# antoinedesbois/Ray-Tracer-Rust

Measured on AMD Instinct MI355X. Metric: Mrays/sec + frame ms, big_bunny.obj @ 1920x1080, higher is better.
Workload: dtype f32

## Files before the change

include/rtx.h:

```cpp
#ifndef RTX_H
#define RTX_H

#include <stddef.h>
#include <stdint.h>

#ifdef __cplusplus
extern "C" {
#endif

#define RTX_ABI_VERSION 3

typedef enum RtxError {
    RTX_OK              =  0,
    RTX_ERR_BAD_ARG     = -1,
    RTX_ERR_NO_DEVICE   = -2,
    RTX_ERR_HIP         = -3,
    RTX_ERR_OOM         = -4,
    RTX_ERR_UNSUPPORTED = -5,
    RTX_ERR_INTERNAL    = -6,
    RTX_ERR_IO          = -7
} RtxError;

#define RTX_ACCEL_BVH    0u
#define RTX_ACCEL_BRUTE  1u
// ... 115 lines not shown
int rtx_render_view_rows(RtxScene *scene, int device, const RtxView *view, uint8_t *out_rgb, RtxStats *stats);
int rtx_render_view_rows_device(RtxScene *scene, int device, const RtxView *view, void *d_rgb, size_t d_bytes,
                                void *stream, uint64_t *d_counters);
int rtx_debug_aimed_nodes(RtxScene *scene, int device, const float eye[3], uint32_t *out_dwords);

typedef struct RtxLight {
    float v0[3], v1[3], v2[3];
    uint32_t nb_light_sample;
} RtxLight;

int rtx_scene_light(const RtxScene *scene, RtxLight *out);
int rtx_render_view_lit(RtxScene *scene, int device, const RtxView *view, const RtxLight *light, uint8_t *out_rgb,
                        RtxPixelShade *out_shade, RtxRayHit *out_hits, RtxStats *stats);
int rtx_render_view_lit_device(RtxScene *scene, int device, const RtxView *view, const RtxLight *light, void *d_rgb,
                               void *d_shade, void *d_hits, void *stream);
int rtx_shade_rays_lit(RtxScene *scene, int device, uint32_t n_pixels, const float *origins, const float *directions,
                       uint32_t flags, const RtxLight *light, RtxPixelShade *out_shade, RtxRayHit *out_hits ,
                       RtxStats *stats);
int rtx_shade_rays_lit_device(RtxScene *scene, int device, uint32_t n_pixels, const void *d_origins, const void *d_directions,
                              uint32_t flags, const RtxLight *light, void *d_shade, void *d_hits ,
                              void *stream);
int rtx_debug_light_points(RtxScene *scene, int device, const RtxLight *light, float *out);

int rtx_render_view_rows_lit(RtxScene *scene, int device, const RtxView *view, const RtxLight *light, uint8_t *out_rgb,
                             RtxStats *stats);
int rtx_render_view_rows_lit_device(RtxScene *scene, int device, const RtxView *view, const RtxLight *light, void *d_rgb,
                                    size_t d_bytes, void *stream, uint64_t *d_counters);
int rtx_debug_light_walk(RtxScene *scene, int device, const RtxLight *light, float *out_tour, float *out_boxes);

int rtx_scene_pose_bound(const RtxScene *scene, float *out_magnitude);
int rtx_scene_pose(RtxScene *scene, int device, const float *v0v1v2, const uint32_t *tie_rank ,
                   uint32_t reference_tree, RtxStats *stats);
int rtx_scene_pose_device(RtxScene *scene, int device, const void *d_v0v1v2, const void *d_tie_rank ,
                          void *stream);
int rtx_trace_rays_posed(RtxScene *scene, int device, uint32_t n_rays, const float *origins, const float *directions,
                         uint32_t flags, RtxRayHit *out_hits, RtxStats *stats);
int rtx_occluded_rays_posed(RtxScene *scene, int device, uint32_t n_rays, const float *origins, const float *targets,
                            uint32_t flags, uint8_t *out_occluded, RtxStats *stats);
int rtx_trace_rays_posed_device(RtxScene *scene, int device, uint32_t n_rays, const void *d_origins, const void *d_directions,
                                uint32_t flags, void *d_hits, void *stream);
int rtx_occluded_rays_posed_device(RtxScene *scene, int device, uint32_t n_rays, const void *d_origins, const void *d_targets,
                                   uint32_t flags, void *d_occluded, void *stream);
int rtx_shade_rays_posed(RtxScene *scene, int device, uint32_t n_pixels, const float *origins, const float *directions,
                         uint32_t flags, const RtxLight *light , RtxPixelShade *out_shade,
                         RtxRayHit *out_hits , RtxStats *stats);
int rtx_shade_rays_posed_device(RtxScene *scene, int device, uint32_t n_pixels, const void *d_origins, const void *d_directions,
                                uint32_t flags, const RtxLight *light , void *d_shade,
                                void *d_hits , void *stream);
int rtx_render_view_posed(RtxScene *scene, int device, const RtxView *view, const RtxLight *light ,
                          uint8_t *out_rgb, RtxPixelShade *out_shade, RtxRayHit *out_hits, RtxStats *stats);
int rtx_render_view_posed_device(RtxScene *scene, int device, const RtxView *view, const RtxLight *light ,
                                 void *d_rgb, void *d_shade, void *d_hits, void *stream);
int rtx_scene_posed_records(const RtxScene *scene, const float *v0v1v2, const uint32_t *tie_rank, uint32_t *out_tris,
                            uint32_t *out_shade, uint32_t *out_nodes);
int rtx_debug_pose(RtxScene *scene, int device, uint32_t *out_tris, uint32_t *out_shade, uint32_t *out_nodes);

int rtx_render_view_rows_posed(RtxScene *scene, int device, const RtxView *view, const RtxLight *light ,
                               uint8_t *out_rgb, RtxStats *stats);
int rtx_render_view_rows_posed_device(RtxScene *scene, int device, const RtxView *view, const RtxLight *light ,
                                      void *d_rgb, size_t d_bytes, void *stream, uint64_t *d_counters);
int rtx_scene_posed_pipeline_records(const RtxScene *scene, const float *v0v1v2, const float eye[3], uint32_t *out_planes,
                                     uint32_t *out_aimed);
int rtx_debug_pose_pipeline(RtxScene *scene, int device, const float eye[3], uint32_t *out_planes, uint32_t *out_aimed);

int rtx_scene_pose_rebuilt(RtxScene *scene, int device, const float *v0v1v2, const uint32_t *tie_rank ,
                           uint32_t reference_tree, RtxStats *stats);
int rtx_scene_pose_rebuilt_device(RtxScene *scene, int device, const void *d_v0v1v2, const void *d_tie_rank ,
                                  void *stream);
int rtx_scene_rebuilt_counts(const RtxScene *scene, uint32_t *out_n_nodes);
int rtx_scene_rebuilt_records(const RtxScene *scene, const float *v0v1v2, const uint32_t *tie_rank, uint64_t *out_keys,
                              uint32_t *out_perm, uint32_t *out_tris, uint32_t *out_shade, uint32_t *out_nodes);
int rtx_scene_rebuilt_aimed(const RtxScene *scene, const float *v0v1v2, const float eye[3], uint32_t *out_aimed);
int rtx_debug_pose_rebuilt(RtxScene *scene, int device, const float eye[3], uint32_t *out_perm, uint32_t *out_tris,
                           uint32_t *out_shade, uint32_t *out_nodes, uint32_t *out_aimed);

#define RTX_WAVE_PROFILE_WORDS 8
int rtx_debug_wave_profile(RtxScene *scene, int device, uint32_t row0, uint32_t nrows, uint64_t *out,
                           size_t out_tiles, uint32_t *tiles_x, uint32_t *tiles_y);

#define RTX_TIMING_RING 64
int rtx_launch_timings(RtxScene *scene, int device, int max_launches, float *schedule_ms, float *shade_ms);

int rtx_debug_tile_descs(RtxScene *scene, int device, uint32_t *out, size_t max_tiles);

const char *rtx_strerror(int err);
int rtx_last_hip_error(void);

int rtx_scene_light_points(const RtxScene *scene, float *out);
int rtx_scene_light_points_for(const RtxScene *scene, const RtxLight *light, float *out);
int rtx_scene_light_order(const RtxScene *scene, uint32_t *out);
int rtx_scene_light_walk_for(const RtxScene *scene, const RtxLight *light, uint32_t *out_order, float *out_boxes,
                             float *out_shaft_delta);
int rtx_scene_gamma_thresholds(const RtxScene *scene, float *out256);
int rtx_scene_normals(const RtxScene *scene, float *out);
int rtx_scene_nodes(const RtxScene *scene, uint32_t *out_dwords , uint32_t *out_tri_order );
int rtx_scene_primary_nodes(const RtxScene *scene, uint32_t *out_dwords , uint32_t *out_own);
int rtx_scene_aimed_nodes(const RtxScene *scene, const float eye[3], uint32_t *out_dwords);
int rtx_scene_ref_nodes(const RtxScene *scene, uint32_t *out_dwords);

void rtxh_camera_new(const float eye[3], const float look_at[3], const float up[3],
                     float u[3], float v[3], float w[3]);
int  rtxh_import_obj(const char *path, float **v0v1v2);
#define RTXH_OBJ_SLASHES   1u
#define RTXH_OBJ_RELATIVE  2u
#define RTXH_OBJ_POLYGONS  4u
#define RTXH_OBJ_MATERIALS 8u
#define RTXH_OBJ_ALL       15u
int  rtxh_import_obj_ex(const char *path, uint32_t flags, float **v0v1v2, float **rgb);
void rtxh_free(void *p);
int  rtxh_ref_leaf_rank(uint32_t n_tris, const float *v0v1v2, uint32_t *out_rank);
void rtxh_gen_samples(uint64_t seed, uint32_t n_pairs, float *out);
int  rtxh_scatter_tiles(uint8_t *frame, uint32_t height, uint32_t width, const uint8_t *packed, uint32_t first_tile,
                        uint32_t tile_stride, uint32_t tile_rows);
int  rtxh_write_png(const char *path, uint32_t width, uint32_t height, const uint8_t *rgb);
int  rtxh_synthetic_mesh(uint64_t seed, uint32_t n_tris, float *out_v0v1v2);

#ifdef __cplusplus
}
#endif
#endif
```

integration/rtx_ffi.rs:

```rust
#![allow(dead_code)]
use std::ffi::CStr;
use std::os::raw::{c_char, c_int, c_void};

pub const RTX_ABI_VERSION: c_int = 3;
pub const RTX_OK: c_int = 0;

#[repr(C)]
#[derive(Clone, Copy, Default)]
pub struct Sample {
    pub s0: f32,
    pub s1: f32,
}

#[repr(C)]
pub struct RtxSceneDesc {
    pub width: u32,
    pub height: u32,
    pub eye: [f32; 3],
    pub u: [f32; 3],
    pub v: [f32; 3],
    pub w: [f32; 3],
    pub distance: f32,
    pub light_v0: [f32; 3],
    pub light_v1: [f32; 3],
// ... 129 lines not shown
                           out_shade: *mut RtxPixelShade, out_hits: *mut RtxRayHit, stats: *mut RtxStats) -> c_int;
    pub fn rtx_render_view_device(scene: *mut RtxScene, device: c_int, view: *const RtxView, d_rgb: *mut c_void,
                                  d_shade: *mut c_void, d_hits: *mut c_void, stream: *mut c_void) -> c_int;
    pub fn rtx_render_view_rows(scene: *mut RtxScene, device: c_int, view: *const RtxView, out_rgb: *mut u8,
                                stats: *mut RtxStats) -> c_int;
    pub fn rtx_render_view_rows_device(scene: *mut RtxScene, device: c_int, view: *const RtxView, d_rgb: *mut c_void,
                                       d_bytes: usize, stream: *mut c_void, d_counters: *mut u64) -> c_int;
    pub fn rtx_scene_light(scene: *const RtxScene, out: *mut RtxLight) -> c_int;
    pub fn rtx_render_view_lit(scene: *mut RtxScene, device: c_int, view: *const RtxView, light: *const RtxLight,
                               out_rgb: *mut u8, out_shade: *mut RtxPixelShade, out_hits: *mut RtxRayHit,
                               stats: *mut RtxStats) -> c_int;
    pub fn rtx_render_view_lit_device(scene: *mut RtxScene, device: c_int, view: *const RtxView, light: *const RtxLight,
                                      d_rgb: *mut c_void, d_shade: *mut c_void, d_hits: *mut c_void,
                                      stream: *mut c_void) -> c_int;
    pub fn rtx_shade_rays_lit(scene: *mut RtxScene, device: c_int, n_pixels: u32, origins: *const f32,
                              directions: *const f32, flags: u32, light: *const RtxLight, out_shade: *mut RtxPixelShade,
                              out_hits: *mut RtxRayHit, stats: *mut RtxStats) -> c_int;
    pub fn rtx_shade_rays_lit_device(scene: *mut RtxScene, device: c_int, n_pixels: u32, d_origins: *const c_void,
                                     d_directions: *const c_void, flags: u32, light: *const RtxLight, d_shade: *mut c_void,
                                     d_hits: *mut c_void, stream: *mut c_void) -> c_int;
    pub fn rtx_scene_pose_bound(scene: *const RtxScene, out_magnitude: *mut f32) -> c_int;
    pub fn rtx_scene_pose(scene: *mut RtxScene, device: c_int, v0v1v2: *const f32, tie_rank: *const u32, reference_tree: u32,
                          stats: *mut RtxStats) -> c_int;
    pub fn rtx_scene_pose_device(scene: *mut RtxScene, device: c_int, d_v0v1v2: *const c_void, d_tie_rank: *const c_void,
                                 stream: *mut c_void) -> c_int;
    pub fn rtx_trace_rays_posed(scene: *mut RtxScene, device: c_int, n_rays: u32, origins: *const f32, directions: *const f32,
                                flags: u32, out_hits: *mut RtxRayHit, stats: *mut RtxStats) -> c_int;
    pub fn rtx_occluded_rays_posed(scene: *mut RtxScene, device: c_int, n_rays: u32, origins: *const f32, targets: *const f32,
                                   flags: u32, out_occluded: *mut u8, stats: *mut RtxStats) -> c_int;
    pub fn rtx_trace_rays_posed_device(scene: *mut RtxScene, device: c_int, n_rays: u32, d_origins: *const c_void,
                                       d_directions: *const c_void, flags: u32, d_hits: *mut c_void,
                                       stream: *mut c_void) -> c_int;
    pub fn rtx_occluded_rays_posed_device(scene: *mut RtxScene, device: c_int, n_rays: u32, d_origins: *const c_void,
                                          d_targets: *const c_void, flags: u32, d_occluded: *mut c_void,
                                          stream: *mut c_void) -> c_int;
    pub fn rtx_shade_rays_posed(scene: *mut RtxScene, device: c_int, n_pixels: u32, origins: *const f32, directions: *const f32,
                                flags: u32, light: *const RtxLight, out_shade: *mut RtxPixelShade, out_hits: *mut RtxRayHit,
                                stats: *mut RtxStats) -> c_int;
    pub fn rtx_shade_rays_posed_device(scene: *mut RtxScene, device: c_int, n_pixels: u32, d_origins: *const c_void,
                                       d_directions: *const c_void, flags: u32, light: *const RtxLight, d_shade: *mut c_void,
                                       d_hits: *mut c_void, stream: *mut c_void) -> c_int;
    pub fn rtx_render_view_posed(scene: *mut RtxScene, device: c_int, view: *const RtxView, light: *const RtxLight,
                                 out_rgb: *mut u8, out_shade: *mut RtxPixelShade, out_hits: *mut RtxRayHit,
                                 stats: *mut RtxStats) -> c_int;
    pub fn rtx_render_view_posed_device(scene: *mut RtxScene, device: c_int, view: *const RtxView, light: *const RtxLight,
                                        d_rgb: *mut c_void, d_shade: *mut c_void, d_hits: *mut c_void,
                                        stream: *mut c_void) -> c_int;
    pub fn rtx_scene_posed_records(scene: *const RtxScene, v0v1v2: *const f32, tie_rank: *const u32, out_tris: *mut u32,
                                   out_shade: *mut u32, out_nodes: *mut u32) -> c_int;
    pub fn rtx_debug_pose(scene: *mut RtxScene, device: c_int, out_tris: *mut u32, out_shade: *mut u32,
                          out_nodes: *mut u32) -> c_int;
    pub fn rtx_render_view_rows_posed(scene: *mut RtxScene, device: c_int, view: *const RtxView, light: *const RtxLight,
                                      out_rgb: *mut u8, stats: *mut RtxStats) -> c_int;
    pub fn rtx_render_view_rows_posed_device(scene: *mut RtxScene, device: c_int, view: *const RtxView, light: *const RtxLight,
                                             d_rgb: *mut c_void, d_bytes: usize, stream: *mut c_void,
                                             d_counters: *mut u64) -> c_int;
    pub fn rtx_scene_posed_pipeline_records(scene: *const RtxScene, v0v1v2: *const f32, eye: *const f32, out_planes: *mut u32,
                                            out_aimed: *mut u32) -> c_int;
    pub fn rtx_debug_pose_pipeline(scene: *mut RtxScene, device: c_int, eye: *const f32, out_planes: *mut u32,
                                   out_aimed: *mut u32) -> c_int;
    pub fn rtx_scene_pose_rebuilt(scene: *mut RtxScene, device: c_int, v0v1v2: *const f32, tie_rank: *const u32,
                                  reference_tree: u32, stats: *mut RtxStats) -> c_int;
    pub fn rtx_scene_pose_rebuilt_device(scene: *mut RtxScene, device: c_int, d_v0v1v2: *const c_void, d_tie_rank: *const c_void,
                                         stream: *mut c_void) -> c_int;
    pub fn rtx_scene_rebuilt_counts(scene: *const RtxScene, out_n_nodes: *mut u32) -> c_int;
    pub fn rtx_scene_rebuilt_records(scene: *const RtxScene, v0v1v2: *const f32, tie_rank: *const u32, out_keys: *mut u64,
                                     out_perm: *mut u32, out_tris: *mut u32, out_shade: *mut u32, out_nodes: *mut u32) -> c_int;
    pub fn rtx_scene_rebuilt_aimed(scene: *const RtxScene, v0v1v2: *const f32, eye: *const f32, out_aimed: *mut u32) -> c_int;
    pub fn rtx_debug_pose_rebuilt(scene: *mut RtxScene, device: c_int, eye: *const f32, out_perm: *mut u32, out_tris: *mut u32,
                                  out_shade: *mut u32, out_nodes: *mut u32, out_aimed: *mut u32) -> c_int;
    pub fn rtx_scene_light_points_for(scene: *const RtxScene, light: *const RtxLight, out: *mut f32) -> c_int;
    pub fn rtx_debug_light_points(scene: *mut RtxScene, device: c_int, light: *const RtxLight, out: *mut f32) -> c_int;
    pub fn rtx_render_view_rows_lit(scene: *mut RtxScene, device: c_int, view: *const RtxView, light: *const RtxLight,
                                    out_rgb: *mut u8, stats: *mut RtxStats) -> c_int;
    pub fn rtx_render_view_rows_lit_device(scene: *mut RtxScene, device: c_int, view: *const RtxView, light: *const RtxLight,
                                           d_rgb: *mut c_void, d_bytes: usize, stream: *mut c_void,
                                           d_counters: *mut u64) -> c_int;
    pub fn rtx_scene_light_walk_for(scene: *const RtxScene, light: *const RtxLight, out_order: *mut u32, out_boxes: *mut f32,
                                    out_shaft_delta: *mut f32) -> c_int;
    pub fn rtx_debug_light_walk(scene: *mut RtxScene, device: c_int, light: *const RtxLight, out_tour: *mut f32,
                                out_boxes: *mut f32) -> c_int;
    pub fn rtx_launch_timings(scene: *mut RtxScene, device: c_int, max_launches: c_int, schedule_ms: *mut f32,
                              shade_ms: *mut f32) -> c_int;
    pub fn rtx_strerror(err: c_int) -> *const c_char;
    pub fn rtx_last_hip_error() -> c_int;
    pub fn rtxh_scatter_tiles(frame: *mut u8, height: u32, width: u32, packed: *const u8, first_tile: u32,
                              tile_stride: u32, tile_rows: u32) -> c_int;
    pub fn rtxh_camera_new(eye: *const f32, look_at: *const f32, up: *const f32, u: *mut f32, v: *mut f32, w: *mut f32);
    pub fn rtxh_ref_leaf_rank(n_tris: u32, v0v1v2: *const f32, out_rank: *mut u32) -> c_int;
}

pub fn check(rc: c_int) -> Result<(), String> {
    if rc == RTX_OK {
        Ok(())
    } else {
        let text = unsafe { CStr::from_ptr(rtx_strerror(rc)) };
        Err(format!("librtx: {} [{}]", text.to_string_lossy(), rc))
    }
}
```

ray-tracer-rust_amd/csrc/rtx_api.cpp:

```cpp
#include <hip/hip_runtime.h>

#include <algorithm>
#include <chrono>
#include <cmath>
#include <cstddef>
#include <cstdio>
#include <cstdlib>
#include <cstring>
#include <initializer_list>
#include <map>
#include <memory>
#include <mutex>
#include <new>
#include <vector>

#include "../../include/rtx.h"
#include "rtx_aim.h"
#include "rtx_device.h"
#include "rtx_light.h"
#include "rtx_planes.h"
#include "rtx_pose.h"
#include "rtx_rebuild.h"
#include "rtx_query.h"
#include "rtx_shade.h"
#include "rtx_tour.h"
#include "rtx_view.h"
#include "scene_prep.h"

namespace {

thread_local int g_last_hip_error = 0;

int hip_rc(hipError_t e)
{
    if (e == hipSuccess) return RTX_OK;
    g_last_hip_error = static_cast<int>(e);
    return e == hipErrorOutOfMemory ? RTX_ERR_OOM : RTX_ERR_HIP;
}

#define RTX_TRY(step)                          \
    do {                                       \
        const int rc_ = (step);                \
        if (rc_ != RTX_OK) return rc_;         \
    } while (0)
#define RTX_HIP(call) RTX_TRY(hip_rc(call))

class DeviceGuard {
public:
    DeviceGuard() = default;
    explicit DeviceGuard(int dev) { (void)set(dev); }
    ~DeviceGuard() { if (ok_) (void)hipSetDevice(prev_); }
    hipError_t set(int dev) { ok_ = hipGetDevice(&prev_) == hipSuccess; return err_ = hipSetDevice(dev); }
    hipError_t status() const { return err_; }
private:
    int prev_ = 0;
    bool ok_ = false;
    hipError_t err_ = hipSuccess;
};

template <class T, hipError_t (*Free)(T)>
class Owned {
public:
    Owned() = default;
    Owned(const Owned &) = delete;
    Owned &operator=(const Owned &) = delete;
    ~Owned() { (void)reset(); }
    hipError_t reset()
    {
        const hipError_t e = h_ ? Free(h_) : hipSuccess;
        h_ = nullptr;
        return e;
    }
    T *put() { return &h_; }
    operator T() const { return h_; }
private:
    T h_ = nullptr;
};
using Stream = Owned<hipStream_t, hipStreamDestroy>;
using Event = Owned<hipEvent_t, hipEventDestroy>;

int mark_busy(Event &e, hipStream_t callers)
{
    if (!e) RTX_HIP(hipEventCreateWithFlags(e.put(), hipEventDisableTiming));
    RTX_HIP(hipEventRecord(e, callers));
    return RTX_OK;
}

int wait_for(const Event &e, hipStream_t stream)
{
    if (e) RTX_HIP(hipStreamWaitEvent(stream, e, 0));
    return RTX_OK;
}

hipError_t alloc_device(void **p, size_t bytes) { return hipMalloc(p, bytes); }
hipError_t alloc_pinned(void **p, size_t bytes) { return hipHostMalloc(p, bytes, hipHostMallocDefault); }

template <hipError_t (*Alloc)(void **, size_t), hipError_t (*Free)(void *)>
class GrowOnly {
public:
    int reserve(size_t bytes)
    {
        if (cap_ >= bytes) return RTX_OK;
        cap_ = 0;
        RTX_HIP(mem_.reset());
        RTX_HIP(Alloc(mem_.put(), bytes));
        cap_ = bytes;
        return RTX_OK;
    }
    size_t capacity() const { return cap_; }
    template <class T>
    T *as() const { return static_cast<T *>(static_cast<void *>(mem_)); }
private:
    Owned<void *, Free> mem_;
    size_t cap_ = 0;
};
using DeviceBuffer = GrowOnly<alloc_device, hipFree>;
using PinnedBuffer = GrowOnly<alloc_pinned, hipHostFree>;

struct Sized { DeviceBuffer &buffer; size_t bytes; };
int reserve_all(std::initializer_list<Sized> list)
{
    for (const Sized &s : list) {
        const int rc = s.buffer.reserve(s.bytes);
        if (rc != RTX_OK) return rc;
    }
    return RTX_OK;
}

struct AimedStream {
    DeviceBuffer nodes, links;
    float eye[3] = {0.0f, 0.0f, 0.0f};
    hipStream_t on = nullptr;
    bool valid = false;
};

struct DeviceGeometry {
    DeviceBuffer nodes, ref_nodes, tris, shade, planes;
    uint32_t n_nodes = 0;
    uint32_t n_ref_nodes = 0;
    AimedStream aimed;
};

class DeviceState {
public:
    explicit DeviceState(int dev) : device(dev) {}
    const int device;
    bool uploaded = false;
    size_t last_tiles = 0;
    unsigned long long launches = 0;
    Stream stream;
    Event ev0, ev1;
    Event ring[RTX_TIMING_RING][3];
    Event q_sorted;
    DeviceGeometry geo;
    DeviceBuffer primary_nodes, samples, lights, light_tour, thr, light_boxes;
    DeviceBuffer d_out, d_counters;
    DeviceBuffer d_redo;
    bool launch_words_ready = false;
    uint32_t words_launches = 0, words_passes = 0;
    PinnedBuffer h_stage;
    struct { DeviceBuffer hits, pix_slot, tiles, chunks, results, acc, ctr, buckets, cut; } ws;
    DeviceBuffer q_first, q_second, q_out;
    struct { DeviceBuffer keys, keys_sorted, index, index_sorted, temp; } q_sort;
    struct {
        DeviceBuffer points, tour, boxes;
        Event used;
    } lit;
    struct {
        DeviceBuffer tri_of, ranges, order;
        bool tables = false;
        DeviceBuffer v, rank;
        DeviceGeometry geo;
        bool valid = false;
        Event used;
        struct {
            DeviceBuffer nodes, ranges, order;
            bool tables = false;
            DeviceBuffer keys, keys_sorted, index, perm, temp;
        } b;
        bool rebuilt = false;
    } pose;
private:
    ~DeviceState() = default;
    friend struct ReleaseOnDevice;
};

struct ReleaseOnDevice {
    void operator()(DeviceState *st) const
    {
        DeviceGuard g(st->device);
        if (g.status() != hipSuccess) return;
        if (st->stream) (void)hipStreamSynchronize(st->stream);
        delete st;
    }
};

struct DeviceSlot {
    std::mutex mu;
    std::unique_ptr<DeviceState, ReleaseOnDevice> st;
};

enum : unsigned { kUsesSort = 1u, kUsesLight = 2u, kUsesPose = 4u };

int wait_for_uses(DeviceState &st, unsigned uses)
{
    if (uses & kUsesSort) RTX_TRY(wait_for(st.q_sorted, st.stream));
    if (uses & kUsesLight) RTX_TRY(wait_for(st.lit.used, st.stream));
    if (uses & kUsesPose) RTX_TRY(wait_for(st.pose.used, st.stream));
    return RTX_OK;
}

int mark_uses(DeviceState &st, unsigned uses, hipStream_t callers)
{
    if (uses & kUsesSort) RTX_TRY(mark_busy(st.q_sorted, callers));
    if (uses & kUsesLight) RTX_TRY(mark_busy(st.lit.used, callers));
    if (uses & kUsesPose) RTX_TRY(mark_busy(st.pose.used, callers));
    return RTX_OK;
}

double wall_ms()
{
    using namespace std::chrono;
    return duration<double, std::milli>(steady_clock::now().time_since_epoch()).count();
}

}

struct RtxScene {
    rtx::PreparedScene prep;
    std::mutex mu;
    rtx::PoseTables pose_tables;
    bool pose_tables_made = false;
    rtx::RebuildTables rebuild_tables;
    bool rebuild_tables_made = false;
    std::map<int, DeviceSlot> dev;
};

namespace {

int device_count_quiet()
{
    int n = 0;
    if (hipGetDeviceCount(&n) != hipSuccess) return 0;
    return n < 0 ? 0 : n;
}

int get_slot(RtxScene *scene, int device, DeviceSlot **out)
{
    if (device < 0 || device >= device_count_quiet()) return RTX_ERR_NO_DEVICE;
    std::lock_guard<std::mutex> lk(scene->mu);
    *out = &scene->dev[device];
    return RTX_OK;
}

int ensure_state(DeviceSlot &slot, int device)
{
    if (!slot.st) slot.st.reset(new (std::nothrow) DeviceState(device));
    return slot.st ? RTX_OK : RTX_ERR_OOM;
}

template <class T>
int upload_vec(DeviceBuffer &dst, const std::vector<T> &v, size_t pad_bytes = 0)
{
    const size_t bytes = v.size() * sizeof(T);
    const int rc = dst.reserve(bytes + pad_bytes ? bytes + pad_bytes : 16);
    if (rc != RTX_OK) return rc;
    if (bytes) RTX_HIP(hipMemcpy(dst.as<void>(), v.data(), bytes, hipMemcpyHostToDevice));
    if (pad_bytes) RTX_HIP(hipMemset(dst.as<char>() + bytes, 0, pad_bytes));
    return RTX_OK;
}

uint32_t kernel_variant()
{
#if RTX_ABLATION
    static const uint32_t v = [] {
        const char *e = std::getenv("RTX_VARIANT");
        return e ? static_cast<uint32_t>(std::atoi(e)) & rtx::kVariantMask : rtx::kDefaultVariant;
    }();
    return v;
#else
    return rtx::kDefaultVariant;
#endif
}

int upload_all(RtxScene *scene, DeviceState &st)
{
    const rtx::PreparedScene &p = scene->prep;
    int rc;
    const float inflate = p.cull_delta;
    DeviceGeometry &g = st.geo;
    if ((rc = upload_vec(g.nodes, rtx::nodes_in_device_order(p.nodes, inflate), sizeof(rtx::NodeRec))) != RTX_OK) return rc;
    if (!p.primary_nodes.empty() &&
        (rc = upload_vec(st.primary_nodes, rtx::nodes_in_device_order(p.primary_nodes, inflate), sizeof(rtx::NodeRec))) != RTX_OK) return rc;
    if (!p.ref_nodes.empty() &&
        (rc = upload_vec(g.ref_nodes, rtx::nodes_in_device_order(p.ref_nodes), sizeof(rtx::NodeRec))) != RTX_OK) return rc;
    g.n_nodes = static_cast<uint32_t>(p.nodes.size());
    g.n_ref_nodes = static_cast<uint32_t>(p.ref_nodes.size());
    if ((rc = upload_vec(g.tris, p.tris, sizeof(rtx::TriRec))) != RTX_OK) return rc;
    if ((rc = upload_vec(g.shade, p.shade)) != RTX_OK) return rc;
    if ((rc = upload_vec(st.samples, p.samples)) != RTX_OK) return rc;
    if ((rc = upload_vec(st.lights, p.light_points)) != RTX_OK) return rc;
    if ((rc = upload_vec(st.light_tour, p.light_tour)) != RTX_OK) return rc;
    if (!p.global_planes.empty() && (rc = upload_vec(g.planes, p.global_planes)) != RTX_OK) return rc;
    if ((rc = upload_vec(st.light_boxes, p.light_boxes)) != RTX_OK) return rc;
    if ((rc = st.thr.reserve(sizeof(p.gamma_thr))) != RTX_OK) return rc;
    RTX_HIP(hipMemcpy(st.thr.as<void>(), p.gamma_thr, sizeof(p.gamma_thr), hipMemcpyHostToDevice));
    if ((rc = st.d_counters.reserve(rtx::kNumCounters * sizeof(unsigned long long))) != RTX_OK) return rc;
    RTX_HIP(hipStreamCreateWithFlags(st.stream.put(), hipStreamNonBlocking));
    RTX_HIP(hipEventCreate(st.ev0.put()));
    RTX_HIP(hipEventCreate(st.ev1.put()));
    for (auto &slot : st.ring)
        for (Event &e : slot) RTX_HIP(hipEventCreate(e.put()));
    st.uploaded = true;
    return RTX_OK;
}

int ensure_uploaded(RtxScene *scene, DeviceSlot &slot)
{
    if (slot.st->uploaded) return RTX_OK;
    const int rc = upload_all(scene, *slot.st);
    if (rc != RTX_OK) slot.st.reset();
    return rc;
}

class Entry {
public:
    enum Need { kLocked, kCurrent, kUploaded };
    Entry(RtxScene *scene, int device, Need need)
    {
        if ((rc = get_slot(scene, device, &slot)) != RTX_OK) return;
        lock_ = std::unique_lock<std::mutex>(slot->mu);
        if ((rc = ensure_state(*slot, device)) != RTX_OK) return;
        if (need >= kCurrent && (rc = make_current()) != RTX_OK) return;
        if (need >= kUploaded) rc = ensure_uploaded(scene, *slot);
    }
    int make_current() { return hip_rc(guard_.set(slot->st->device)); }
    DeviceState &state() const { return *slot->st; }
    int rc = RTX_ERR_INTERNAL;
    DeviceSlot *slot = nullptr;
private:
    std::unique_lock<std::mutex> lock_;
    DeviceGuard guard_;
};

int geometry_of(DeviceState &st, bool posed, DeviceGeometry **out)
{
    *out = &st.geo;
    if (!posed) return RTX_OK;
    if (!st.pose.valid) return RTX_ERR_BAD_ARG;
    *out = &st.pose.geo;
    return RTX_OK;
}

rtx::DeviceScene device_scene(const RtxScene *scene, const DeviceState &st, const DeviceGeometry &g)
{
    const rtx::PreparedScene &p = scene->prep;
    rtx::DeviceScene S;
    S.nodes = g.nodes.as<const rtx::NodeRec>();
    S.primary_nodes = st.primary_nodes.capacity() ? st.primary_nodes.as<const rtx::NodeRec>() : st.geo.nodes.as<const rtx::NodeRec>();
    S.light_tour = st.light_tour.as<const float>();
    S.n_wide = 0u;
    S.ref_nodes = g.ref_nodes.as<const rtx::NodeRec>();
    S.n_ref_nodes = g.n_ref_nodes;
    S.tris = g.tris.as<const rtx::TriRec>();
    S.shade = g.shade.as<const rtx::ShadeRec>();
    S.samples = st.samples.as<const float2>();
    S.light_points = st.lights.as<const float>();
    S.planes = g.planes.as<const rtx::TriRec>();
    S.gamma_thr = st.thr.as<const float>();
    S.light_boxes = st.light_boxes.as<const float>();
    S.shaft_delta = p.shaft_delta;
    S.n_nodes = g.n_nodes;
    S.n_samples = p.n_samples;
    S.width = p.width;
    S.height = p.height;
    S.nb_ray = p.nb_ray;
    S.nb_light = p.nb_light_sample;
    S.n_spheres = p.n_spheres;
    S.n_global = p.n_global;
    std::memcpy(S.eye, p.eye, 12);
    std::memcpy(S.cu, p.cam_u, 12);
    std::memcpy(S.cv, p.cam_v, 12);
    std::memcpy(S.cw, p.cam_w, 12);
    S.distance = p.distance;
    S.cut_max_nodes = rtx::kCutMaxNodes;
    S.n_prims = static_cast<uint32_t>(p.tris.size());
    S.j1_mode = 0u;
// ... 5 lines not shown
        if (m == 1u || ((m == 2u || m == 3u) && p.n_spheres == 0u)) S.j1_mode = m;
    }
#endif
    return S;
}

int reserve_stream_ws(DeviceState &st, const rtx::DeviceScene &S, const rtx::TileSpec &ts, rtx::StreamWorkspace *ws, bool *used)
{
    *used = (kernel_variant() & (rtx::kVariantStream | rtx::kVariantProbe)) != 0u;
    if (!*used) return RTX_OK;
    const rtx::StreamWorkspaceBytes need = rtx::stream_workspace_bytes(S, ts, kernel_variant());
    const int rc = reserve_all({{st.ws.hits, need.hits}, {st.ws.pix_slot, need.pix_slot}, {st.ws.tiles, need.tiles},
                                {st.ws.chunks, need.chunks}, {st.ws.results, need.results}, {st.ws.acc, need.acc},
                                {st.ws.ctr, need.ctr}, {st.ws.buckets, need.buckets}, {st.ws.cut, need.cut}});
    if (rc != RTX_OK) return rc;
    st.last_tiles = need.tiles / sizeof(rtx::TileDesc);
    *ws = rtx::StreamWorkspace{st.ws.hits.as<rtx::HitRec>(), st.ws.pix_slot.as<uint32_t>(), st.ws.tiles.as<rtx::TileDesc>(),
                               st.ws.chunks.as<uint2>(), st.ws.results.as<float>(), st.ws.acc.as<float>(),
                               st.ws.ctr.as<uint32_t>(), st.ws.buckets.as<uint32_t>(), st.ws.cut.as<rtx::CutEntry>()};
    return RTX_OK;
}

uint32_t tiles_rows(uint32_t height, uint32_t first_tile, uint32_t tile_stride, uint32_t tile_rows)
{
    if (!tile_rows || !tile_stride) return 0;
    uint64_t rows = 0;
    for (uint64_t t = first_tile; t * tile_rows < height; t += tile_stride) {
        const uint64_t r0 = t * tile_rows;
        rows += (height - r0 < tile_rows) ? (height - r0) : tile_rows;
    }
    return static_cast<uint32_t>(rows);
}

void fill_stats(RtxStats *s, uint64_t primary_rays, uint32_t shadow_rays_per_hit, const unsigned long long *c,
                double kernel_ms, double total_ms)
{
    std::memset(s, 0, sizeof *s);
    s->primary_rays = primary_rays;
    s->primary_hits = c[0];
    s->shadow_rays = c[0] * shadow_rays_per_hit;
    s->rays = s->primary_rays + s->shadow_rays;
    s->box_tests = c[1];
    s->tri_tests = c[2];
    s->wave_node_visits = c[3];
    s->wave_tri_visits = c[4];
    s->redo_tiles = c[5];
    s->kernel_ms = kernel_ms;
    s->total_ms = total_ms;
}

struct Timed {
    explicit Timed(RtxStats *s) : stats(s) {}
    RtxStats *const stats;
    const double t0 = wall_ms();
    unsigned long long *counters(const DeviceState &st) const { return stats ? st.d_counters.as<unsigned long long>() : nullptr; }
    int empty() const
    {
        const unsigned long long none[rtx::kNumCounters] = {0};
        if (stats) fill_stats(stats, 0, 0, none, 0.0, wall_ms() - t0);
        return RTX_OK;
    }
    int begin(const DeviceState &st) const
    {
        if (stats) RTX_HIP(hipMemsetAsync(counters(st), 0, rtx::kNumCounters * sizeof(unsigned long long), st.stream));
        RTX_HIP(hipEventRecord(st.ev0, st.stream));
        return RTX_OK;
    }
    int end(const DeviceState &st) const { return hip_rc(hipEventRecord(st.ev1, st.stream)); }
    int gather(const DeviceState &st, uint64_t primary_rays, uint32_t shadow_rays_per_hit) const
    {
        unsigned long long c[rtx::kNumCounters] = {0};
        if (stats) RTX_HIP(hipMemcpyAsync(c, counters(st), sizeof c, hipMemcpyDeviceToHost, st.stream));
        RTX_HIP(hipStreamSynchronize(st.stream));
        if (!stats) return RTX_OK;
        float ms = 0.0f;
        RTX_HIP(hipEventElapsedTime(&ms, st.ev0, st.ev1));
        fill_stats(stats, primary_rays, shadow_rays_per_hit, c, ms, wall_ms() - t0);
        return RTX_OK;
    }
};

template <class Before>
int render_launch(DeviceState &st, const rtx::DeviceScene &S, const rtx::TileSpec &ts, uint8_t *d_out,
                  unsigned long long *d_counters, unsigned long long *d_wave_prof, hipStream_t stream, Before before)
{
    int rc;
    const size_t redo_cap = st.d_redo.capacity(), buckets_cap = st.ws.buckets.capacity();
    if ((rc = st.d_redo.reserve(rtx::trace_redo_bytes(S, ts))) != RTX_OK) return rc;
    rtx::StreamWorkspace ws{};
    bool use_ws = false;
    if (!d_wave_prof && (rc = reserve_stream_ws(st, S, ts, &ws, &use_ws)) != RTX_OK) return rc;
    if ((rc = before()) != RTX_OK) return rc;
    const Event *slot = st.ring[st.launches % RTX_TIMING_RING];
    hipEvent_t phases[3] = {slot[0], slot[1], slot[2]};
    const bool two_pass = use_ws && (kernel_variant() & rtx::kVariantProbe) != 0u && ts.local_rows != 0u;
    if (two_pass && (!st.launch_words_ready || st.d_redo.capacity() != redo_cap || st.ws.buckets.capacity() != buckets_cap)) {
        RTX_HIP(rtx::zero_launch_words(st.d_redo.as<uint32_t>(), ws, stream));
        st.words_launches = st.words_passes = 0;
    }
    if (ts.local_rows) st.launch_words_ready = false;
    RTX_HIP(rtx::launch_trace_shade(S, ts, d_out, st.d_redo.as<uint32_t>(), use_ws ? &ws : nullptr, d_counters, d_wave_prof,
                                    kernel_variant(), stream, d_wave_prof ? nullptr : phases, st.words_launches, st.words_passes));
    if (two_pass) {
        st.launch_words_ready = true;
        ++st.words_launches;
        st.words_passes += S.nb_ray;
    }
    if (!d_wave_prof && ts.local_rows) ++st.launches;
    return RTX_OK;
}

int launch_on(RtxScene *scene, DeviceSlot &slot, const rtx::TileSpec &ts, const Timed &timed)
{
    RTX_TRY(ensure_uploaded(scene, slot));
    DeviceState &st = *slot.st;
    const size_t bytes = static_cast<size_t>(ts.local_rows) * scene->prep.width * 3u;
    RTX_TRY(st.d_out.reserve(bytes ? bytes : 16));
    RTX_TRY(render_launch(st, device_scene(scene, st, st.geo), ts, st.d_out.as<uint8_t>(), timed.counters(st), nullptr, st.stream,
                          [&] { return timed.begin(st); }));
    return timed.end(st);
}


uint32_t tree_root(const rtx::PreparedScene &p, size_t n_nodes)
{
    return (p.n_global != 0u && n_nodes > 2u) ? 2u : 0u;
}
uint32_t tree_root(const rtx::PreparedScene &p) { return tree_root(p, p.nodes.size()); }

float origin_bound(const RtxScene *scene) { return scene->prep.cull_delta * 0x1p19f; }

rtxq::KeyBox query_key_box(const rtx::PreparedScene &p)
{
    rtxq::KeyBox box{};
    if (p.nodes.empty()) return box;
    const rtx::NodeRec &root = p.nodes[tree_root(p)];
    for (int a = 0; a < 3; ++a) {
        const float extent = root.bmax[a] - root.bmin[a];
        const float scale = static_cast<float>(1u << rtxq::kMortonBitsPerAxis) / extent;
        box.lo[a] = root.bmin[a];
        box.scale[a] = (extent > 0.0f && scale > 0.0f && scale < 0x1p100f) ? scale : 0.0f;
    }
    return box;
}

int reserve_query_sort(DeviceState &st, uint32_t n, rtxq::SortBuffers *sort)
{
    const size_t words = static_cast<size_t>(n) * sizeof(uint32_t);
    size_t temp = 0;
    RTX_HIP(rtxq::sort_temp_bytes(n, &temp));
    const int rc = reserve_all({{st.q_sort.keys, words}, {st.q_sort.keys_sorted, words}, {st.q_sort.index, words},
                                {st.q_sort.index_sorted, words}, {st.q_sort.temp, temp ? temp : 16}});
    if (rc != RTX_OK) return rc;
    *sort = rtxq::SortBuffers{st.q_sort.keys.as<uint32_t>(), st.q_sort.keys_sorted.as<uint32_t>(), st.q_sort.index.as<uint32_t>(),
                              st.q_sort.index_sorted.as<uint32_t>(), st.q_sort.temp.as<void>(), st.q_sort.temp.capacity()};
    return RTX_OK;
}

static_assert(sizeof(RtxRayHit) == 32, "closest_kernel writes a hit as two 16-byte words");
static_assert(sizeof(RtxPixelShade) == 16, "shade_kernel writes a pixel as one 16-byte word");
static_assert(sizeof(RtxView) == sizeof(rtxv::ViewBlock) && alignof(RtxView) == 4, "view_kernel is handed an RtxView");
constexpr uint32_t kQueryFlags = RTX_RAYS_KEEP_ORDER | RTX_RAYS_FORCE_REGROUP;

uint32_t shade_ray_count(const RtxScene *scene, uint32_t n_pixels)
{
    const uint64_t n = static_cast<uint64_t>(n_pixels) * scene->prep.nb_ray;
    return n <= rtxq::kMaxRays ? static_cast<uint32_t>(n) : 0u;
}

constexpr int kBatchOuts = 3;
struct BatchArgs {
    rtx::DeviceScene S;
    uint32_t n;
    const float *first, *second;
    const RtxView *view;
    rtxq::KeyBox box;
    float origin_bound;
    const rtxq::SortBuffers *sort;
    void *out[kBatchOuts];
    unsigned long long *counters;
    hipStream_t stream;
};

template <bool Occlusion>
hipError_t launch_queried(const BatchArgs &a)
{
    return rtxq::launch_query(a.S, Occlusion, a.n, a.first, a.second, a.box, a.origin_bound, a.sort, a.out[0], a.counters, a.stream);
}

hipError_t launch_shaded(const BatchArgs &a)
{
    return rtxs::launch_shade(a.S, a.n, a.first, a.second, a.box, a.origin_bound, a.sort, a.out[0], a.out[1], a.counters, a.stream);
}

enum { kViewShade, kViewHits, kViewRgb };

hipError_t launch_viewed(const BatchArgs &a)
{
    rtxv::ViewBlock v;
    std::memcpy(&v, a.view, sizeof v);
    return rtxv::launch_view(a.S, v, a.origin_bound, a.out[kViewRgb], a.out[kViewShade], a.out[kViewHits], a.counters, a.stream);
}
// ... 397 lines not shown

int shade_host(RtxScene *scene, int device, uint32_t n_pixels, const float *origins, const float *directions, uint32_t flags,
               const Lit *lit, bool posed, RtxPixelShade *shade, RtxRayHit *hits, RtxStats *stats)
{
    if (!shade_args_ok(scene, origins, directions, shade, flags, n_pixels)) return RTX_ERR_BAD_ARG;
    return batch_host(scene, device, shade_batch(scene, n_pixels, flags, lit, posed, hits != nullptr), origins, directions,
                      {shade, hits, nullptr}, stats);
}

int shade_device(RtxScene *scene, int device, uint32_t n_pixels, const void *d_origins, const void *d_directions, uint32_t flags,
                 const Lit *lit, bool posed, void *d_shade, void *d_hits, void *stream)
{
    if (!shade_args_ok(scene, d_origins, d_directions, d_shade, flags, n_pixels) || !aligned16(d_shade, d_hits)) return RTX_ERR_BAD_ARG;
    return batch_device(scene, device, shade_batch(scene, n_pixels, flags, lit, posed, d_hits != nullptr), d_origins, d_directions,
                        {d_shade, d_hits, nullptr}, stream);
}


bool eye_in_pipeline_range(const RtxScene *scene, const float eye[3])
{
    const float bound = origin_bound(scene);
    for (int k = 0; k < 3; ++k)
        if (!(std::fabs(eye[k]) <= bound)) return false;
    return true;
}

bool view_rows_args_ok(const RtxScene *scene, const RtxView *v, const void *out)
{
    if (!scene || !v || !out || !frame_ok(v)) return false;
    if (v->x0 != 0u || v->nx != v->width) return false;
    return static_cast<uint64_t>(v->y0) + v->ny <= v->height;
}

int reserve_aimed(const RtxScene *scene, DeviceGeometry &g)
{
    if (scene->prep.primary_nodes.empty()) return RTX_OK;
    AimedStream &a = g.aimed;
    const size_t n = g.n_nodes;
    const size_t had = a.nodes.capacity();
    const int rc = reserve_all({{a.nodes, (n + 1u) * sizeof(rtx::NodeDev)}, {a.links, n * sizeof(rtxa::AimLink)}});
    if (rc != RTX_OK || a.nodes.capacity() != had) a.valid = false;
    return rc;
}

const rtx::NodeRec *aimed_stream(const RtxScene *scene, const DeviceGeometry &g)
{
    return (scene->prep.primary_nodes.empty() ? g.nodes : g.aimed.nodes).as<const rtx::NodeRec>();
}

int aim_at(const RtxScene *scene, DeviceGeometry &g, const float eye[3], hipStream_t stream)
{
    const rtx::PreparedScene &p = scene->prep;
    if (p.primary_nodes.empty()) return RTX_OK;
    AimedStream &a = g.aimed;
    if (a.valid && a.on == stream && std::memcmp(a.eye, eye, 12) == 0) return RTX_OK;
    a.valid = false;
    const uint32_t n = g.n_nodes;
    RTX_HIP(hipMemsetAsync(a.nodes.as<rtx::NodeDev>() + n, 0, sizeof(rtx::NodeDev), stream));
    RTX_HIP(rtxa::launch_aim(g.nodes.as<const rtx::NodeDev>(), n, tree_root(p, n), eye, a.links.as<rtxa::AimLink>(),
                             a.nodes.as<rtx::NodeDev>(), stream));
    std::memcpy(a.eye, eye, 12);
    a.on = stream;
    a.valid = true;
    return RTX_OK;
}

template <class Before>
int view_rows_launch(RtxScene *scene, DeviceState &st, DeviceGeometry &g, const RtxView &v, uint8_t *d_out,
                     unsigned long long *d_counters, hipStream_t stream, Before before, const Lit *lit, float shaft_delta)
{
    RTX_TRY(reserve_aimed(scene, g));
    if (lit) RTX_TRY(reserve_light(scene, st, *lit, true));
    rtx::DeviceScene S = device_scene(scene, st, g);
    if (lit) light_swap(st, *lit, true, shaft_delta, &S);
    S.width = v.width;
    S.height = v.height;
    std::memcpy(S.eye, v.eye, 12);
    std::memcpy(S.cu, v.u, 12);
    std::memcpy(S.cv, v.v, 12);
    std::memcpy(S.cw, v.w, 12);
    S.distance = v.distance;
    S.primary_nodes = aimed_stream(scene, g);
    const rtx::TileSpec ts{v.y0, v.ny, v.ny, v.ny};
    return render_launch(st, S, ts, d_out, d_counters, nullptr, stream, [&]() -> int {
        RTX_TRY(before());
        RTX_TRY(aim_at(scene, g, v.eye, stream));
        return lit ? light_launch(scene, st, *lit, true, stream) : RTX_OK;
    });
}

int view_rows_supported(const RtxScene *scene, const RtxView *view, const Lit *lit, float *shaft_delta)
{
    if (!eye_in_pipeline_range(scene, view->eye)) return RTX_ERR_UNSUPPORTED;
    return lit ? lit_rows_margin(scene, *lit, shaft_delta) : RTX_OK;
}

int view_rows_host(RtxScene *scene, int device, const RtxView *view, const Lit *lit, bool posed, uint8_t *out_rgb, RtxStats *stats)
{
    if (!view_rows_args_ok(scene, view, out_rgb)) return RTX_ERR_BAD_ARG;
    const Timed timed(stats);
    if (view->ny == 0u) return timed.empty();
    float shaft_delta = 0.0f;
    RTX_TRY(view_rows_supported(scene, view, lit, &shaft_delta));
    Entry e(scene, device, Entry::kUploaded);
    if (e.rc != RTX_OK) return e.rc;
    DeviceState &st = e.state();
    const RtxView v = *view;
    const size_t bytes = static_cast<size_t>(v.ny) * v.width * 3u;
    RTX_TRY(st.d_out.reserve(bytes));
    DeviceGeometry *geo;
    RTX_TRY(geometry_of(st, posed, &geo));
    RTX_TRY(wait_for_uses(st, uses_of(lit, posed)));
    RTX_TRY(view_rows_launch(scene, st, *geo, v, st.d_out.as<uint8_t>(), timed.counters(st), st.stream, [&] { return timed.begin(st); },
                             lit, shaft_delta));
    RTX_TRY(timed.end(st));
    RTX_HIP(hipMemcpyAsync(out_rgb, st.d_out.as<void>(), bytes, hipMemcpyDeviceToHost, st.stream));
    return timed.gather(st, static_cast<uint64_t>(v.ny) * v.width * scene->prep.nb_ray, lit ? lit->count : scene->prep.nb_light_sample);
}

int view_rows_device(RtxScene *scene, int device, const RtxView *view, const Lit *lit, bool posed, void *d_rgb, size_t d_bytes,
                     void *stream, uint64_t *d_counters)
{
    if (!view_rows_args_ok(scene, view, d_rgb)) return RTX_ERR_BAD_ARG;
    if (d_bytes < static_cast<size_t>(view->ny) * view->width * 3u) return RTX_ERR_BAD_ARG;
    if (view->ny == 0u) return RTX_OK;
    float shaft_delta = 0.0f;
    RTX_TRY(view_rows_supported(scene, view, lit, &shaft_delta));
    Entry e(scene, device, Entry::kUploaded);
    if (e.rc != RTX_OK) return e.rc;
    DeviceGeometry *geo;
    RTX_TRY(geometry_of(e.state(), posed, &geo));
    RTX_TRY(view_rows_launch(scene, e.state(), *geo, *view, static_cast<uint8_t *>(d_rgb), reinterpret_cast<unsigned long long *>(d_counters),
                             static_cast<hipStream_t>(stream), [] { return static_cast<int>(RTX_OK); }, lit, shaft_delta));
    return mark_uses(e.state(), uses_of(lit, posed), static_cast<hipStream_t>(stream));
}

void posed_pipeline_on_host(RtxScene *scene, const float *pose, const float *eye, rtx::TriRec *planes, rtx::NodeRec *aimed)
{
    const rtx::PreparedScene &p = scene->prep;
    const rtx::PoseTables &t = pose_tables_of(scene);
    std::vector<rtx::TriRec> tris(p.tris.size());
    std::vector<rtx::NodeRec> nodes(aimed ? p.nodes.size() : 0u);
    rtx::posed_records(p, t, pose, nullptr, tris.data(), nullptr, aimed ? nodes.data() : nullptr);
    if (planes)
        for (uint32_t i = 0; i < p.n_global; ++i) rtx::global_plane_statement(tris[i], planes + i);
    if (!aimed) return;
    if (!p.primary_nodes.empty()) {
        std::vector<rtx::NodeRec> out;
        rtx::stream_nearest_first(nodes, tree_root(p), eye, out);
        nodes.swap(out);
    }
    std::memcpy(aimed, nodes.data(), nodes.size() * sizeof(rtx::NodeRec));
}

std::vector<rtx::NodeRec> aimed_on_host(const rtx::PreparedScene &p, const float eye[3])
{
    std::vector<rtx::NodeRec> moved(p.nodes);
    const float inflate = p.cull_delta;
    for (rtx::NodeRec &n : moved)
        for (int k = 0; k < 3; ++k) {
            n.bmin[k] = n.bmin[k] - inflate;
            n.bmax[k] = n.bmax[k] + inflate;
        }
    if (p.primary_nodes.empty()) return moved;
    std::vector<rtx::NodeRec> out;
    rtx::stream_nearest_first(moved, tree_root(p), eye, out);
// ... 219 lines not shown
        RTX_HIP(g.status());
        const auto &n = need[kv.second];
        int rc = ensure_state(*kv.second, kv.first);
        if (rc != RTX_OK) return rc;
        if ((rc = kv.second->st->d_out.reserve(n.first ? n.first : 16)) != RTX_OK) return rc;
        if ((rc = kv.second->st->h_stage.reserve(n.second ? n.second : 16)) != RTX_OK) return rc;
    }
    unsigned long long total[rtx::kNumCounters] = {0};
    std::vector<unsigned long long> counters(static_cast<size_t>(n_devices) * rtx::kNumCounters, 0ull);
    std::vector<float> share_ms(static_cast<size_t>(n_devices), 0.0f);
    for (int j = 0; j < n_devices; ++j) {
        Share &sh = shares[j];
        if (!sh.spec.local_rows) continue;
        DeviceGuard g(devices[j]);
        if (g.status() != hipSuccess) return fail(hip_rc(g.status()));
        const int rc = launch_on(scene, *sh.slot, sh.spec, Timed(stats));
        if (rc != RTX_OK) return fail(rc);
        launched.push_back(devices[j]);
        DeviceState &st = *sh.slot->st;
        hipError_t e = hipMemcpyAsync(st.h_stage.as<uint8_t>() + sh.stage_offset, st.d_out.as<void>(), sh.spec.local_rows * row_bytes,
                                      hipMemcpyDeviceToHost, st.stream);
        if (e == hipSuccess && stats)
            e = hipMemcpyAsync(&counters[static_cast<size_t>(j) * rtx::kNumCounters], st.d_counters.as<void>(),
                               rtx::kNumCounters * sizeof(unsigned long long), hipMemcpyDeviceToHost, st.stream);
        if (e != hipSuccess) return fail(hip_rc(e));
        if (stats && unique.size() != static_cast<size_t>(n_devices)) {
            if ((e = hipStreamSynchronize(st.stream)) != hipSuccess || (e = hipEventElapsedTime(&share_ms[j], st.ev0, st.ev1)) != hipSuccess)
                return fail(hip_rc(e));
        }
    }
    double kernel_ms = 0.0;
    for (auto &kv : unique) {
        DeviceGuard g(kv.first);
        if (g.status() != hipSuccess) return fail(hip_rc(g.status()));
        const hipError_t e = hipStreamSynchronize(kv.second->st->stream);
        if (e != hipSuccess) return fail(hip_rc(e));
    }
    for (int j = 0; j < n_devices; ++j) {
        const Share &sh = shares[j];
        if (!sh.spec.local_rows) continue;
        rtxh_scatter_tiles(out_rgb, H, W, sh.slot->st->h_stage.as<uint8_t>() + sh.stage_offset, static_cast<uint32_t>(j), static_cast<uint32_t>(n_devices), tile_rows);
        if (stats) {
            if (unique.size() == static_cast<size_t>(n_devices)) {
                DeviceGuard g(devices[j]);
                float ms = 0.0f;
                if (g.status() == hipSuccess && hipEventElapsedTime(&ms, sh.slot->st->ev0, sh.slot->st->ev1) == hipSuccess) share_ms[j] = ms;
            }
            for (int k = 0; k < rtx::kNumCounters; ++k) total[k] += counters[static_cast<size_t>(j) * rtx::kNumCounters + k];
        }
    }
    if (stats) {
        std::map<DeviceSlot *, double> per_device;
        for (int j = 0; j < n_devices; ++j) per_device[shares[j].slot] += share_ms[j];
        for (auto &kv : per_device) kernel_ms = std::max(kernel_ms, kv.second);
        fill_stats(stats, static_cast<uint64_t>(H) * W * scene->prep.nb_ray, scene->prep.nb_light_sample, total, kernel_ms, wall_ms() - t0);
    }
    return RTX_OK;
}

uint32_t rtx_tiles_rows(const RtxScene *scene, uint32_t first_tile, uint32_t tile_stride, uint32_t tile_rows)
{
    return scene ? tiles_rows(scene->prep.height, first_tile, tile_stride, tile_rows) : 0;
}

size_t rtx_tiles_bytes(const RtxScene *scene, uint32_t first_tile, uint32_t tile_stride, uint32_t tile_rows)
{
    return scene ? static_cast<size_t>(tiles_rows(scene->prep.height, first_tile, tile_stride, tile_rows)) *
                       scene->prep.width * 3u
                 : 0;
}

int rtx_render_tiles_device(RtxScene *scene, int device, uint32_t first_tile, uint32_t tile_stride,
                            uint32_t tile_rows, void *d_out_rgb, size_t d_out_bytes, void *stream,
                            uint64_t *d_counters)
{
    if (!scene || !d_out_rgb || !tile_rows || !tile_stride) return RTX_ERR_BAD_ARG;
    const uint32_t rows = tiles_rows(scene->prep.height, first_tile, tile_stride, tile_rows);
    if (static_cast<size_t>(rows) * scene->prep.width * 3u > d_out_bytes) return RTX_ERR_BAD_ARG;
    if (static_cast<uint64_t>(first_tile) * tile_rows > 0xFFFFFFFFull ||
        static_cast<uint64_t>(tile_stride) * tile_rows > 0xFFFFFFFFull) return RTX_ERR_BAD_ARG;
    Entry e(scene, device, Entry::kUploaded);
    if (e.rc != RTX_OK) return e.rc;
    const rtx::TileSpec ts{first_tile * tile_rows, tile_rows, tile_stride * tile_rows, rows};
    return render_launch(e.state(), device_scene(scene, e.state(), e.state().geo), ts, static_cast<uint8_t *>(d_out_rgb),
                         reinterpret_cast<unsigned long long *>(d_counters), nullptr, static_cast<hipStream_t>(stream),
                         [] { return static_cast<int>(RTX_OK); });
}

int rtx_trace_rays(RtxScene *scene, int device, uint32_t n_rays, const float *origins, const float *directions,
                   uint32_t flags, RtxRayHit *out_hits, RtxStats *stats)
{
    if (!query_args_ok(scene, origins, directions, out_hits, flags, n_rays)) return RTX_ERR_BAD_ARG;
    return batch_host(scene, device, query_batch(false, n_rays, flags, false), origins, directions, {out_hits, nullptr, nullptr}, stats);
}

int rtx_occluded_rays(RtxScene *scene, int device, uint32_t n_rays, const float *origins, const float *targets,
                      uint32_t flags, uint8_t *out_occluded, RtxStats *stats)
{
    if (!query_args_ok(scene, origins, targets, out_occluded, flags, n_rays)) return RTX_ERR_BAD_ARG;
    return batch_host(scene, device, query_batch(true, n_rays, flags, false), origins, targets, {out_occluded, nullptr, nullptr}, stats);
}

int rtx_trace_rays_device(RtxScene *scene, int device, uint32_t n_rays, const void *d_origins, const void *d_directions,
                          uint32_t flags, void *d_hits, void *stream)
{
    if (!query_args_ok(scene, d_origins, d_directions, d_hits, flags, n_rays) || !aligned16(d_hits)) return RTX_ERR_BAD_ARG;
    return batch_device(scene, device, query_batch(false, n_rays, flags, false), d_origins, d_directions, {d_hits, nullptr, nullptr}, stream);
}

int rtx_occluded_rays_device(RtxScene *scene, int device, uint32_t n_rays, const void *d_origins, const void *d_targets,
                             uint32_t flags, void *d_occluded, void *stream)
{
    if (!query_args_ok(scene, d_origins, d_targets, d_occluded, flags, n_rays)) return RTX_ERR_BAD_ARG;
    return batch_device(scene, device, query_batch(true, n_rays, flags, false), d_origins, d_targets, {d_occluded, nullptr, nullptr}, stream);
}

int rtx_shade_rays(RtxScene *scene, int device, uint32_t n_pixels, const float *origins, const float *directions,
                   uint32_t flags, RtxPixelShade *out_shade, RtxRayHit *out_hits, RtxStats *stats)
{
    return shade_host(scene, device, n_pixels, origins, directions, flags, nullptr, false, out_shade, out_hits, stats);
}

int rtx_shade_rays_device(RtxScene *scene, int device, uint32_t n_pixels, const void *d_origins, const void *d_directions,
                          uint32_t flags, void *d_shade, void *d_hits, void *stream)
{
    return shade_device(scene, device, n_pixels, d_origins, d_directions, flags, nullptr, false, d_shade, d_hits, stream);
}

int rtx_scene_view(const RtxScene *scene, RtxView *out)
{
    if (!scene || !out) return RTX_ERR_BAD_ARG;
    const rtx::PreparedScene &p = scene->prep;
    std::memset(out, 0, sizeof *out);
    out->width = out->nx = p.width;
    out->height = out->ny = p.height;
    std::memcpy(out->eye, p.eye, 12);
    std::memcpy(out->u, p.cam_u, 12);
    std::memcpy(out->v, p.cam_v, 12);
    std::memcpy(out->w, p.cam_w, 12);
    out->distance = p.distance;
    return RTX_OK;
}

int rtx_render_view(RtxScene *scene, int device, const RtxView *view, uint8_t *out_rgb, RtxPixelShade *out_shade,
                    RtxRayHit *out_hits, RtxStats *stats)
{
    return view_host(scene, device, view, nullptr, false, out_rgb, out_shade, out_hits, stats);
}

int rtx_render_view_device(RtxScene *scene, int device, const RtxView *view, void *d_rgb, void *d_shade, void *d_hits,
                           void *stream)
{
    return view_device(scene, device, view, nullptr, false, d_rgb, d_shade, d_hits, stream);
}

int rtx_scene_light(const RtxScene *scene, RtxLight *out)
{
    if (!scene || !out) return RTX_ERR_BAD_ARG;
    const rtx::PreparedScene &p = scene->prep;
    std::memcpy(out->v0, p.light_v, 12);
    std::memcpy(out->v1, p.light_v + 3, 12);
    std::memcpy(out->v2, p.light_v + 6, 12);
    out->nb_light_sample = p.nb_light_sample;
    return RTX_OK;
}

int rtx_render_view_lit(RtxScene *scene, int device, const RtxView *view, const RtxLight *light, uint8_t *out_rgb,
                        RtxPixelShade *out_shade, RtxRayHit *out_hits, RtxStats *stats)
{
// ... 342 lines not shown
    if (!scene || !v0v1v2 || (out_aimed && !eye)) return RTX_ERR_BAD_ARG;
    try {
        posed_pipeline_on_host(const_cast<RtxScene *>(scene), v0v1v2, eye, reinterpret_cast<rtx::TriRec *>(out_planes),
                               reinterpret_cast<rtx::NodeRec *>(out_aimed));
    } catch (...) {
        return RTX_ERR_OOM;
    }
    return RTX_OK;
}

int rtx_debug_pose_pipeline(RtxScene *scene, int device, const float eye[3], uint32_t *out_planes, uint32_t *out_aimed)
{
    if (!scene || (out_aimed && !eye)) return RTX_ERR_BAD_ARG;
    Entry e(scene, device, Entry::kUploaded);
    if (e.rc != RTX_OK) return e.rc;
    DeviceState &st = e.state();
    DeviceGeometry *g;
    RTX_TRY(geometry_of(st, true, &g));
    if (st.pose.rebuilt && out_aimed) return RTX_ERR_BAD_ARG;
    const size_t n = scene->prep.nodes.size(), n_global = scene->prep.n_global;
    RTX_TRY(wait_for_uses(st, kUsesPose));
    if (out_planes && n_global)
        RTX_HIP(hipMemcpyAsync(out_planes, g->planes.as<void>(), n_global * sizeof(rtx::TriRec), hipMemcpyDeviceToHost, st.stream));
    if (out_aimed && n) {
        RTX_TRY(reserve_aimed(scene, *g));
        g->aimed.valid = false;
        RTX_TRY(aim_at(scene, *g, eye, st.stream));
    }
    return read_back_nodes(st, aimed_stream(scene, *g), n, out_aimed);
}

int rtx_debug_wave_profile(RtxScene *scene, int device, uint32_t row0, uint32_t nrows, uint64_t *out,
                           size_t out_tiles, uint32_t *tiles_x, uint32_t *tiles_y)
{
    if (!scene || !tiles_x || !tiles_y) return RTX_ERR_BAD_ARG;
    const uint32_t H = scene->prep.height;
    if (row0 > H || nrows > H - row0 || nrows == 0) return RTX_ERR_BAD_ARG;
#if !RTX_ABLATION
    (void)device; (void)out; (void)out_tiles;
    return RTX_ERR_UNSUPPORTED;
#else
    Entry en(scene, device, Entry::kUploaded);
    if (en.rc != RTX_OK) return en.rc;
    DeviceState &st = en.state();
    const rtx::DeviceScene S = device_scene(scene, st, st.geo);
    *tiles_x = rtx::trace_tiles_x(S, kernel_variant());
    *tiles_y = (nrows + 7u) / 8u;
    const size_t n = static_cast<size_t>(*tiles_x) * *tiles_y;
    if (!out) return RTX_OK;
    if (out_tiles < n) return RTX_ERR_BAD_ARG;
    int rc = st.d_out.reserve(static_cast<size_t>(nrows) * scene->prep.width * 3u);
    if (rc != RTX_OK) return rc;
    unsigned long long *d_prof = nullptr;
    const size_t prof_bytes = n * rtx::kWaveProfWords * sizeof(unsigned long long);
    RTX_HIP(hipMalloc(reinterpret_cast<void **>(&d_prof), prof_bytes));
    const rtx::TileSpec ts{row0, nrows, nrows, nrows};
    rc = render_launch(st, S, ts, st.d_out.as<uint8_t>(), nullptr, d_prof, st.stream,
                       [&] { return hip_rc(hipMemsetAsync(d_prof, 0, prof_bytes, st.stream)); });
    if (rc == RTX_OK) rc = hip_rc(hipMemcpyAsync(out, d_prof, prof_bytes, hipMemcpyDeviceToHost, st.stream));
    if (rc == RTX_OK) rc = hip_rc(hipStreamSynchronize(st.stream));
    (void)hipFree(d_prof);
    if (rc != RTX_OK) return rc;
    for (size_t t = 0; t < n; ++t)
        out[rtx::kWaveProfWords * t + 2] = ~out[rtx::kWaveProfWords * t + 2];
    return RTX_OK;
#endif
}

int rtx_debug_tile_descs(RtxScene *scene, int device, uint32_t *out, size_t max_tiles)
{
    if (!scene) return RTX_ERR_BAD_ARG;
    Entry e(scene, device, Entry::kLocked);
    if (e.rc != RTX_OK) return e.rc;
    const DeviceState &st = e.state();
    if (!out) return static_cast<int>(st.last_tiles);
    const int rc = e.make_current();
    if (rc != RTX_OK) return rc;
    const size_t n = st.last_tiles < max_tiles ? st.last_tiles : max_tiles;
    RTX_HIP(hipDeviceSynchronize());
    if (n) RTX_HIP(hipMemcpy(out, st.ws.tiles.as<void>(), n * sizeof(rtx::TileDesc), hipMemcpyDeviceToHost));
    return static_cast<int>(n);
}

int rtx_launch_timings(RtxScene *scene, int device, int max_launches, float *schedule_ms, float *shade_ms)
{
    if (!scene || max_launches < 0 || !schedule_ms || !shade_ms) return RTX_ERR_BAD_ARG;
    Entry e(scene, device, Entry::kCurrent);
    if (e.rc != RTX_OK) return e.rc;
    const DeviceState &st = e.state();
    unsigned long long n = st.launches < RTX_TIMING_RING ? st.launches : RTX_TIMING_RING;
    if (n > static_cast<unsigned long long>(max_launches)) n = static_cast<unsigned long long>(max_launches);
    for (unsigned long long i = 0; i < n; ++i) {
        const Event *ev = st.ring[(st.launches - n + i) % RTX_TIMING_RING];
        RTX_HIP(hipEventSynchronize(ev[2]));
        RTX_HIP(hipEventElapsedTime(&schedule_ms[i], ev[0], ev[1]));
        RTX_HIP(hipEventElapsedTime(&shade_ms[i], ev[1], ev[2]));
    }
    return static_cast<int>(n);
}

int rtx_scene_light_points(const RtxScene *scene, float *out)
{
    if (!scene || !out) return RTX_ERR_BAD_ARG;
    std::memcpy(out, scene->prep.light_points.data(), scene->prep.light_points.size() * sizeof(float));
    return RTX_OK;
}

int rtx_scene_light_order(const RtxScene *scene, uint32_t *out)
{
    if (!scene || !out) return RTX_ERR_BAD_ARG;
    std::memcpy(out, scene->prep.light_order.data(), scene->prep.light_order.size() * sizeof(uint32_t));
    return RTX_OK;
}

int rtx_scene_gamma_thresholds(const RtxScene *scene, float *out256)
{
    if (!scene || !out256) return RTX_ERR_BAD_ARG;
    std::memcpy(out256, scene->prep.gamma_thr, sizeof scene->prep.gamma_thr);
    return RTX_OK;
}

int rtx_scene_normals(const RtxScene *scene, float *out)
{
    if (!scene || !out) return RTX_ERR_BAD_ARG;
    for (size_t i = 0; i < scene->prep.shade.size(); ++i) std::memcpy(out + 3 * i, scene->prep.shade[i].normal, 12);
    return RTX_OK;
}

int rtx_scene_ref_nodes(const RtxScene *scene, uint32_t *out_dwords)
{
    if (!scene || !out_dwords) return RTX_ERR_BAD_ARG;
    std::memcpy(out_dwords, scene->prep.ref_nodes.data(), scene->prep.ref_nodes.size() * sizeof(rtx::NodeRec));
    return RTX_OK;
}

int rtx_scene_primary_nodes(const RtxScene *scene, uint32_t *out_dwords, uint32_t *out_own)
{
    if (!scene) return RTX_ERR_BAD_ARG;
    const bool own = !scene->prep.primary_nodes.empty();
    const std::vector<rtx::NodeRec> &v = own ? scene->prep.primary_nodes : scene->prep.nodes;
    if (out_dwords) std::memcpy(out_dwords, v.data(), v.size() * sizeof(rtx::NodeRec));
    if (out_own) *out_own = own ? 1u : 0u;
    return RTX_OK;
}

int rtx_scene_nodes(const RtxScene *scene, uint32_t *out_dwords, uint32_t *out_tri_order)
{
    if (!scene) return RTX_ERR_BAD_ARG;
    if (out_dwords)
        std::memcpy(out_dwords, scene->prep.nodes.data(), scene->prep.nodes.size() * sizeof(rtx::NodeRec));
    if (out_tri_order)
        for (size_t i = 0; i < scene->prep.tris.size(); ++i) out_tri_order[i] = scene->prep.tris[i].idx;
    return RTX_OK;
}

}
```

ray-tracer-rust_amd/csrc/rtx_device.h:

```cpp
#pragma once

#include <hip/hip_runtime.h>

#include <cstdint>

#include "scene_prep.h"

#ifndef RTX_ABLATION
#define RTX_ABLATION 0
#endif

namespace rtx {

struct DeviceScene {
    const NodeRec  *nodes;
    const NodeRec  *primary_nodes;
    const float    *light_tour;
    const NodeRec  *ref_nodes;
    const TriRec   *tris;
    const ShadeRec *shade;
    const TriRec   *planes;
    const float2   *samples;
    const float    *light_points;
    const float    *gamma_thr;
    const float    *light_boxes;
    uint32_t n_nodes, n_ref_nodes, n_samples, n_wide;
    uint32_t width, height;
    uint32_t nb_ray, nb_light;
    uint32_t n_global;
    uint32_t n_spheres;
    float eye[3], cu[3], cv[3], cw[3];
    float distance;
    float shaft_delta;
    uint32_t cut_max_nodes;
    uint32_t n_prims;
    uint32_t j1_mode;
};
constexpr uint32_t kCutMaxNodes = 1u << 16;

struct TileSpec {
    uint32_t first_row;
    uint32_t tile_rows;
    uint32_t tile_stride_rows;
    uint32_t local_rows;
};

struct TileDesc {
    uint32_t first;
    uint32_t n_hit;
    uint32_t flags;
    uint32_t pad;
};
struct HitRec {
    float p[3], n[3], rgb[3], pad[3];
};
static_assert(sizeof(TileDesc) == 16 && sizeof(HitRec) == 48, "stream record sizes");
struct CutEntry {
    uint32_t begin, end;
    NodeDev  root;
};
static_assert(sizeof(CutEntry) == 40, "CutEntry is ten dwords");
constexpr uint32_t kCutWords = sizeof(CutEntry) / 4u;
#ifndef RTX_MAX_CUT
#define RTX_MAX_CUT 16
#endif
constexpr uint32_t kMaxCut = RTX_MAX_CUT;
struct StreamWorkspace {
    HitRec   *hits;
    uint32_t *pix_slot;
    TileDesc *tiles;
    uint2    *chunks;
    float    *results;
    float    *acc;
    uint32_t *ctr;
    uint32_t *buckets;
    CutEntry *cut;
};
constexpr uint32_t kCutInnerFlag = 1u << 29, kCutEndMask = (1u << 26) - 1u;
constexpr uint32_t kCutStreamRecords = kMaxCut + 1u;
__host__ __device__ inline size_t cut_stream_offset(size_t tiles)
{
    return (tiles * kMaxCut * sizeof(CutEntry) + 63u) & ~static_cast<size_t>(63u);
}
struct StreamWorkspaceBytes { size_t hits, pix_slot, tiles, chunks, results, acc, ctr, buckets, cut; };
static_assert(kMaxCut >= 1u && kMaxCut <= 51u && kCutWords * kMaxCut <= 512u, "RTX_MAX_CUT: 1 .. 51 (one staged word per work-item of 512)");
constexpr uint32_t kTileCutShift = 8u;
constexpr uint32_t kTileCompactHits = 8u;
constexpr uint32_t kTileChunk0Kept = 4u;
StreamWorkspaceBytes stream_workspace_bytes(const DeviceScene &S, const TileSpec &ts, uint32_t variant);
constexpr uint32_t kCostBuckets = 64u;
constexpr uint32_t kStreamCtrWords = 4u;

constexpr int kNumCounters = 8;


constexpr uint32_t kVariantStream = 8u;
constexpr uint32_t kVariantPacked = 16u;
constexpr uint32_t kVariantProbe = 32u;
constexpr uint32_t kVariantMask = 63u;
constexpr uint32_t kDefaultVariant = kVariantProbe | 1u;

constexpr size_t kWaveProfWords = 8;
uint32_t trace_tiles_x(const DeviceScene &S, uint32_t variant);
constexpr uint32_t kQueueRedoCount = 0u, kQueueNextTile = 1u, kQueueHeader = 4u, kQueueSlotStride = 2u;
size_t trace_redo_bytes(const DeviceScene &S, const TileSpec &ts);
hipError_t launch_trace_shade(const DeviceScene &S, const TileSpec &ts, uint8_t *d_out, uint32_t *d_redo,
                              const StreamWorkspace *ws, unsigned long long *d_counters,
                              unsigned long long *d_wave_prof, uint32_t variant, hipStream_t stream,
                              hipEvent_t *phase_events = nullptr, uint32_t launch_no = 0u, uint32_t pass_no = 0u);
hipError_t zero_launch_words(uint32_t *d_redo, const StreamWorkspace &ws, hipStream_t stream);

}
```

ray-tracer-rust_amd/csrc/rtx_kernel.hip:

```cpp
#include <cstdlib>
#include <type_traits>
#include "rtx_traverse.hpp"
#include "rtx_pass_helpers.hpp"
#include "rtx_pass_schedule.hpp"
#include "rtx_pass_order.hpp"
#include "rtx_pass_shade.hpp"

namespace rtx {

template <bool COUNT, bool SPHERES = false>
__global__ void __launch_bounds__(64) reference_tiles_kernel(DeviceScene S, TileSpec ts, uint32_t tiles_x,
                                                              uint8_t *__restrict__ out,
                                                              const uint32_t *__restrict__ redo,
                                                              unsigned long long *__restrict__ counters,
                                                              bool tile_blocks = false)
{
    const TriRec RTX_CONSTANT *tris = (const TriRec RTX_CONSTANT *)S.tris;
    const bool have_ref = S.n_ref_nodes != 0u;
    const NodeRec RTX_CONSTANT *stream = (const NodeRec RTX_CONSTANT *)(have_ref ? S.ref_nodes : S.nodes);
    const uint32_t n_stream = have_ref ? S.n_ref_nodes : S.n_nodes;
    const uint32_t lane = threadIdx.x;
    const uint32_t n_redo = __builtin_amdgcn_readfirstlane(redo[kQueueRedoCount]);
    WaveCounters wc;
    unsigned long long primary_hits = 0;
    for (uint32_t q = blockIdx.x; q < n_redo; q += gridDim.x) {
        const uint32_t tid = __builtin_amdgcn_readfirstlane(redo[kQueueHeader + q]);
        uint32_t px, py, ly;
        uint32_t tile_x, tile_y;
        tile_xy(tid, tiles_x, tile_blocks, tile_x, tile_y);
        const bool in_frame = tile_pixel(S, ts, tile_x, tile_y, lane, px, py, ly);
        float acc_r = 0.0f, acc_g = 0.0f, acc_b = 0.0f;
        const float denom = (float)(S.nb_ray * S.nb_light);
        for (uint32_t r = 0; r < S.nb_ray; ++r) {
            float dx, dy, dz, t;
            uint32_t idx;
            primary_ray(S, in_frame, px, py, r, dx, dy, dz);
            closest_hit_reference<COUNT, SPHERES>(stream, tris, S.shade, n_stream, have_ref, in_frame, S.eye[0], S.eye[1], S.eye[2],
                                         dx, dy, dz, t, idx, wc);
            const bool hit = in_frame && idx != kNone;
            const unsigned long long hit_mask = ballot(hit);
            if (hit_mask == 0ull) continue;
            if (COUNT) primary_hits += __popcll(hit_mask);
            float hx = 0.0f, hy = 0.0f, hz = 0.0f, nx = 0.0f, ny = 0.0f, nz = 0.0f, cr = 0.0f, cg = 0.0f, cb = 0.0f;
            if (hit) {
                hx = S.eye[0] + t * dx;
                hy = S.eye[1] + t * dy;
                hz = S.eye[2] + t * dz;
                const ShadeRec sh = S.shade[idx];
                hit_normal<SPHERES>(sh, hx, hy, hz, nx, ny, nz);
                cr = sh.rgb[0]; cg = sh.rgb[1]; cb = sh.rgb[2];
            }
            for (uint32_t i = 0; i < S.nb_light; ++i) {
                const float *lp = S.light_points + 3u * (r * S.nb_light + i);
                const float vx = lp[0] - hx, vy = lp[1] - hy, vz = lp[2] - hz;
                const float dist_light = sqrtf(vx * vx + vy * vy + vz * vz);
                const float sx = vx / dist_light, sy = vy / dist_light, sz = vz / dist_light;
                float st;
                uint32_t sidx;
                closest_hit_reference<COUNT, SPHERES>(stream, tris, S.shade, n_stream, have_ref, hit, hx, hy, hz, sx, sy, sz,
                                             st, sidx, wc);
                const float lnd = fabsf(nx * sx + ny * sy + nz * sz);
                bool lit = true;
                if (sidx != kNone) {
                    const float qx = hx - (hx + st * sx), qy = hy - (hy + st * sy), qz = hz - (hz + st * sz);
                    lit = sqrtf(qx * qx + qy * qy + qz * qz) > dist_light;
                }
                if (hit && lit) {
                    acc_r = acc_r + ((cr * lnd) / denom);
                    acc_g = acc_g + ((cg * lnd) / denom);
                    acc_b = acc_b + ((cb * lnd) / denom);
                }
            }
        }
        if (in_frame) store_pixel(S, out, px, ly, acc_r, acc_g, acc_b);
    }
    if (COUNT && lane == 0) flush_counters<COUNT>(counters, primary_hits, wc);
}


namespace {

#ifndef RTX_SPLIT_SHARE_PERCENT
#define RTX_SPLIT_SHARE_PERCENT 100
#endif
constexpr float kSplitShare = RTX_SPLIT_SHARE_PERCENT * 0.01f;
float split_share()
{
#if RTX_ABLATION
    static const float v = [] {
        const char *e = getenv("RTX_SPLIT_SHARE");
        const float x = e ? strtof(e, nullptr) : 0.0f;
        return x > 0.0f ? x : kSplitShare;
    }();
    return v;
#else
    return kSplitShare;
#endif
}

template <bool COUNT, bool FAST, bool SPHERES>
hipError_t launch_probe(const DeviceScene &S, const TileSpec &ts, uint8_t *d_out, uint32_t *d_redo,
                        const StreamWorkspace &W, unsigned long long *d_counters, hipStream_t stream, hipEvent_t *ev,
                        uint32_t launch_no, uint32_t pass_no)
{
#ifndef RTX_SHADE_NW
#define RTX_SHADE_NW 8
#endif
    constexpr int NW = RTX_SHADE_NW;
    const bool whole = S.n_nodes > S.cut_max_nodes;
    const auto probe = whole ? probe_kernel<COUNT, FAST, SPHERES, true> : probe_kernel<COUNT, FAST, SPHERES, false>;
    const auto shade = whole ? shade_tiles_kernel<COUNT, FAST, NW, SPHERES, true> : shade_tiles_kernel<COUNT, FAST, NW, SPHERES, false>;
    const uint32_t batch = S.nb_light < kMaxLightBatch ? (S.nb_light ? S.nb_light : 1u) : kMaxLightBatch;
#if RTX_ABLATION
    const size_t lds_bytes = (static_cast<size_t>(lds_floats(batch)) + (S.j1_mode == 1u ? kJ1WindowWords : 0u)) * sizeof(float);
#else
    const size_t lds_bytes = static_cast<size_t>(lds_floats(batch)) * sizeof(float);
#endif
    const uint32_t tiles_x = (S.width + 7u) / 8u, tiles_y = (ts.local_rows + 7u) / 8u;
    const uint32_t n_tiles = numbered_tiles(tiles_x, tiles_y);
    static thread_local int cached_dev = -1, cached_blocks = 0;
    static thread_local size_t cached_lds = 0;
    static thread_local bool cached_whole = false;
    int dev = 0;
    hipError_t e = hipGetDevice(&dev);
    if (e != hipSuccess) return e;
    if (dev != cached_dev || lds_bytes != cached_lds || whole != cached_whole) {
        int per_cu = 0, cus = 0;
        if ((e = hipOccupancyMaxActiveBlocksPerMultiprocessor(&per_cu, shade, 64 * NW, lds_bytes)) != hipSuccess) return e;
        if ((e = hipDeviceGetAttribute(&cus, hipDeviceAttributeMultiprocessorCount, dev)) != hipSuccess) return e;
        cached_blocks = (per_cu > 0 ? per_cu : 1) * (cus > 0 ? cus : 1);
        cached_dev = dev;
        cached_lds = lds_bytes;
        cached_whole = whole;
    }
    if (n_tiles > kJobTileMask) return hipErrorInvalidValue;
    const uint64_t most_jobs = (uint64_t)n_tiles * kMaxTileParts;
    const uint32_t grid = most_jobs < static_cast<uint64_t>(cached_blocks) ? (uint32_t)most_jobs : static_cast<uint32_t>(cached_blocks);
    uint32_t *const queue = d_redo + (launch_no & 1u) * kQueueSlotStride;
    uint32_t *const next_redo_count = d_redo + ((launch_no + 1u) & 1u) * kQueueSlotStride + kQueueRedoCount;
    for (uint32_t r = 0; r < S.nb_ray; ++r) {
        const uint32_t hist_set = (pass_no + r) & 1u;
        const StreamWorkspace Wp = counting_set(W, hist_set);
        hipLaunchKernelGGL(probe, dim3(512u * ((n_tiles + 511u) / 512u)), dim3(64 * kProbeWaves), 0, stream,
                           S, ts, tiles_x, n_tiles, r, Wp, d_out, queue, d_counters);
        if (whole) hipLaunchKernelGGL(count_classes_kernel, dim3((n_tiles + 1023u) / 1024u), dim3(1024), 0, stream, n_tiles, Wp);
        hipLaunchKernelGGL(order_tiles_kernel, dim3((n_tiles + 1023u) / 1024u), dim3(1024), 0, stream, n_tiles, W, grid, split_share(),
                           hist_set, whole ? 0u : grid, queue, next_redo_count);
        if (ev && r == 0u && (e = hipEventRecord(ev[1], stream)) != hipSuccess) return e;
        hipLaunchKernelGGL(shade, dim3(grid), dim3(64 * NW), lds_bytes, stream, S, ts, batch, tiles_x, n_tiles, r, W, d_out, queue, d_counters);
        if ((e = hipGetLastError()) != hipSuccess) return e;
    }
    hipLaunchKernelGGL((reference_tiles_kernel<COUNT, SPHERES>), dim3(n_tiles < 1024u ? n_tiles : 1024u), dim3(64), 0, stream,
                       S, ts, tiles_x, d_out, queue, d_counters, true);
    return hipGetLastError();
}

}

#if RTX_ABLATION
#include "rtx_ablation_kernels.hpp"
#endif

uint32_t trace_tiles_x(const DeviceScene &S, uint32_t) { return (S.width + 7u) / 8u; }

hipError_t zero_launch_words(uint32_t *d_redo, const StreamWorkspace &W, hipStream_t stream)
{
    hipLaunchKernelGGL(reset_kernel, dim3(1), dim3(256), 0, stream, d_redo, 0u, kQueueSlotStride + kQueueHeader, W.buckets, kOrderList);
    return hipGetLastError();
}

size_t trace_redo_bytes(const DeviceScene &S, const TileSpec &ts)
{
    return sizeof(uint32_t) * (kQueueSlotStride + kQueueHeader + static_cast<size_t>(numbered_tiles((S.width + 7u) / 8u, (ts.local_rows + 7u) / 8u)));
}

StreamWorkspaceBytes stream_workspace_bytes(const DeviceScene &S, const TileSpec &ts, uint32_t variant)
{
    const bool streamed = (variant & kVariantStream) != 0u, probe = (variant & kVariantProbe) != 0u;
    const size_t tiles = probe ? numbered_tiles((S.width + 7u) / 8u, (ts.local_rows + 7u) / 8u)
                               : static_cast<size_t>((S.width + 7u) / 8u) * ((ts.local_rows + 7u) / 8u);
    const size_t pixels = tiles * 64u;
    StreamWorkspaceBytes b;
    b.hits = pixels * sizeof(HitRec);
    b.pix_slot = pixels * sizeof(uint32_t);
    b.tiles = tiles * sizeof(TileDesc);
    b.chunks = streamed ? (pixels * S.nb_light / 64u + tiles + 1u) * sizeof(uint2) : 0u;
    b.results = streamed ? pixels * (S.nb_light ? S.nb_light : 1u) * sizeof(float) : 0u;
    b.acc = S.nb_ray > 1u ? pixels * 3u * sizeof(float) : 0u;
    b.ctr = kStreamCtrWords * sizeof(uint32_t);
    b.buckets = probe ? (kOrderList + tiles * kMaxTileParts) * sizeof(uint32_t) : 0u;
    b.cut = probe ? cut_stream_offset(tiles) + tiles * kCutStreamRecords * sizeof(NodeDev) : 0u;
    return b;
}

static hipError_t launch_dispatch(const DeviceScene &S, const TileSpec &ts, uint8_t *d_out, uint32_t *d_redo,
                                  const StreamWorkspace *ws, unsigned long long *d_counters,
                                  unsigned long long *d_wave_prof, uint32_t variant, hipStream_t stream, hipEvent_t *ev,
                                  uint32_t launch_no, uint32_t pass_no)
{
    auto two_pass = [&](auto fast) {
        constexpr bool FAST = decltype(fast)::value;
        const bool count = d_counters != nullptr, spheres = S.n_spheres != 0u;
        const auto launch = count ? (spheres ? launch_probe<true, FAST, true> : launch_probe<true, FAST, false>)
                                  : (spheres ? launch_probe<false, FAST, true> : launch_probe<false, FAST, false>);
        return launch(S, ts, d_out, d_redo, *ws, d_counters, stream, ev, launch_no, pass_no);
    };
#if RTX_ABLATION
    if (!((variant & kVariantProbe) && ws && !d_wave_prof))
        return launch_dispatch_ablation(S, ts, d_out, d_redo, ws, d_counters, d_wave_prof, variant, stream);
    if (!(variant & 1u)) return two_pass(std::false_type{});
#else
    if (variant != kDefaultVariant || !ws || d_wave_prof) return hipErrorInvalidValue;
#endif
    return two_pass(std::true_type{});
}

hipError_t launch_trace_shade(const DeviceScene &S, const TileSpec &ts, uint8_t *d_out, uint32_t *d_redo,
                              const StreamWorkspace *ws, unsigned long long *d_counters,
                              unsigned long long *d_wave_prof, uint32_t variant, hipStream_t stream,
                              hipEvent_t *phase_events, uint32_t launch_no, uint32_t pass_no)
{
    if (ts.local_rows == 0) return hipSuccess;
    hipError_t e;
    if (phase_events && (e = hipEventRecord(phase_events[0], stream)) != hipSuccess) return e;
    const bool probe = (variant & kVariantProbe) && ws && !d_wave_prof;
    if (phase_events && !probe && (e = hipEventRecord(phase_events[1], stream)) != hipSuccess) return e;
    e = launch_dispatch(S, ts, d_out, d_redo, ws, d_counters, d_wave_prof, variant, stream, probe ? phase_events : nullptr, launch_no, pass_no);
    if (e != hipSuccess) return e;
    if (phase_events && (e = hipEventRecord(phase_events[2], stream)) != hipSuccess) return e;
    return hipSuccess;
}

}

#define RTX_SW_STR2(x) #x
#define RTX_SW_STR(x) RTX_SW_STR2(x)
#define RTX_SW(x) " " #x "=" RTX_SW_STR(x)
extern "C" __attribute__((used, visibility("hidden"))) const char rtx_build_switches_text[] = "rtx-build-switches:"
    RTX_SW(RTX_CLAIM_RUN_LOG) RTX_SW(RTX_CUT_DRAW_MIN) RTX_SW(RTX_CUT_UNION_MIN) RTX_SW(RTX_LIGHT_BATCH) RTX_SW(RTX_MAX_CUT)
    RTX_SW(RTX_PACKED_WAVES_PER_SIMD) RTX_SW(RTX_PROBE_VISIT_SCALE) RTX_SW(RTX_PROBE_WAVES_PER_SIMD)
    RTX_SW(RTX_SHADE_CUT_WAVES_PER_SIMD) RTX_SW(RTX_SHADE_NW) RTX_SW(RTX_SHADE_WAVES_PER_SIMD)
    RTX_SW(RTX_SPLIT_SHARE_PERCENT) RTX_SW(RTX_TILE_PARTS_MAX) RTX_SW(RTX_WAVES_PER_SIMD)
    RTX_SW(RTX_EXPERIMENT_TIMELINE) RTX_SW(RTX_EXPERIMENT_PHASES) RTX_SW(RTX_EXPERIMENT_PROBE_PHASES) RTX_SW(RTX_ABLATION);
#undef RTX_SW
```

ray-tracer-rust_amd/csrc/rtx_pass_schedule.hpp:

```cpp
#pragma once
#include "rtx_probes.hpp"
#include "rtx_pass_helpers.hpp"

namespace rtx {

__device__ __forceinline__ uint32_t cost_class(unsigned long long cost)
{
    if (cost == 0ull) return 0u;
    if (cost > 0x7FFFFFFFull) cost = 0x7FFFFFFFull;
    const uint32_t c = (uint32_t)cost;
    const uint32_t lz = 31u - (uint32_t)__clz((int)c);
    const uint32_t half = lz ? (c >> (lz - 1u)) & 1u : 0u;
    const uint32_t k = 2u * lz + half + 1u;
    return k < kCostBuckets ? k : kCostBuckets - 1u;
}

constexpr uint32_t kChunkFixedCost = 8u;


#ifndef RTX_CUT_DRAW_MIN
#define RTX_CUT_DRAW_MIN 1
#endif
constexpr bool kCutEntriesUsed = RTX_ABLATION != 0;
constexpr uint32_t kProbeWaves = 1u;
#ifndef RTX_PROBE_WAVES_PER_SIMD
#define RTX_PROBE_WAVES_PER_SIMD 8
#endif
#ifndef RTX_PROBE_VISIT_SCALE
#define RTX_PROBE_VISIT_SCALE 6u
#endif

struct Shaft {
    float inv[6], off[6];
    uint32_t lower, upper;
};
constexpr float kShaftS0 = -0x1p-8f, kShaftS1 = 1.0f + 0x1p-8f;

__device__ __forceinline__ void shaft_constraint(Shaft &sh, uint32_t c, float o, float g, float delta)
{
    const bool usable = fabsf(g) >= 0x1p-40f && fabsf(g) <= 0x1p60f;
    const float inv = __builtin_amdgcn_rcpf(g);
    sh.inv[c] = usable ? inv : 0.0f;
    sh.off[c] = usable ? (((c & 1u) ? delta : -delta) - o) * inv : 0.0f;
    const bool positive = g > 0.0f;
    const bool is_lower = usable && (((c & 1u) == 0u) == positive);
    if (is_lower) sh.lower |= 1u << c;
    if (usable && !is_lower) sh.upper |= 1u << c;
}

__device__ __forceinline__ bool shaft_meets(const Shaft &sh, const NodeDev &b)
{
    const float plane[6] = {b.lox, b.hix, b.loy, b.hiy, b.loz, b.hiz};
    float s_lo = kShaftS0, s_hi = kShaftS1;
#pragma unroll
    for (uint32_t c = 0; c < 6u; ++c) {
        const float q = __builtin_fmaf(plane[c], sh.inv[c], sh.off[c]);
        s_lo = fmaxf(s_lo, (sh.lower >> c) & 1u ? q : kShaftS0);
        s_hi = fminf(s_hi, (sh.upper >> c) & 1u ? q : kShaftS1);
    }
    return !(s_lo > s_hi);
}

#define RTX_DPP_REDUCE(name, insn)                                                                                          \
    __device__ __forceinline__ float name(float v)                                                                          \
    {                                                                                                                       \
        asm volatile("s_nop 1\n\t" insn " %0, %0, %0 row_shr:1 row_mask:0xf bank_mask:0xf\n\t"                              \
                     "s_nop 1\n\t" insn " %0, %0, %0 row_shr:2 row_mask:0xf bank_mask:0xf\n\t"                              \
                     "s_nop 1\n\t" insn " %0, %0, %0 row_shr:4 row_mask:0xf bank_mask:0xf\n\t"                              \
                     "s_nop 1\n\t" insn " %0, %0, %0 row_shr:8 row_mask:0xf bank_mask:0xf\n\t"                              \
                     "s_nop 1\n\t" insn " %0, %0, %0 row_bcast:15 row_mask:0xa bank_mask:0xf\n\t"                           \
                     "s_nop 1\n\t" insn " %0, %0, %0 row_bcast:31 row_mask:0xc bank_mask:0xf\n\t"                           \
                     "s_nop 1" : "+v"(v));                                                                                  \
        return __int_as_float(__builtin_amdgcn_readlane(__float_as_int(v), 63));                                            \
    }
RTX_DPP_REDUCE(wave_min, "v_min_f32_dpp")
RTX_DPP_REDUCE(wave_max, "v_max_f32_dpp")
#undef RTX_DPP_REDUCE
__device__ __forceinline__ float uniform(float v)
{
    return __int_as_float(__builtin_amdgcn_readfirstlane(__float_as_int(v)));
}
__device__ __forceinline__ uint32_t wave_sum(uint32_t v)
{
#pragma unroll
    for (int m = 32; m >= 1; m >>= 1) v += __shfl_xor(v, m);
    return v;
}

#if RTX_ABLATION
#include "rtx_j1_ablation.hpp"
#endif

template <bool FAST, bool SPHERES>
__device__ __forceinline__ uint32_t probe_cut_walk(const NodeRec RTX_CONSTANT *nodes, const TriRec RTX_CONSTANT *tris,
                                                             const ShadeRec *shade, const uint32_t *l_entries, uint32_t n_cut,
                                                             uint32_t n_global, const float *light_point, bool hit, float hx, float hy,
                                                             float hz)
{
    const float vx = light_point[0] - hx, vy = light_point[1] - hy, vz = light_point[2] - hz;
    float dist_light, sx, sy, sz;
    (void)length_and_direction(vx, vy, vz, dist_light, sx, sy, sz);
    LaneRay sr = make_ray(hit, hx, hy, hz, sx, sy, sz);
    sr.limit = dist_light;
    WaveCounters probe;
    uint32_t first_entry = 0u;
    (void)any_hit_cut<true, FAST, SPHERES>(nodes, tris, shade, l_entries, n_cut, sr, probe, n_global, false, first_entry);
    return (uint32_t)(probe.node_visits + probe.tri_visits);
}

__device__ __forceinline__ uint32_t shaft_cut_binary(const NodeDev *__restrict__ nodes, uint32_t root, const Shaft &sh,
                                                     CutEntry *__restrict__ out, NodeDev *__restrict__ out_stream,
                                                     uint32_t *__restrict__ l_front, CutEntry *__restrict__ l_entries,
                                                     uint32_t lane, uint32_t &weight)
{
    auto stream_record = [](uint32_t at, bool leaf, NodeDev nd) {
        if (!leaf) { nd.info = kLeafFlag | kCutInnerFlag | nd.link; nd.link = at; }
        return nd;
    };
    uint32_t my = root, n_front = 1u, n_out = 0u, w = 0u;
    const float inf = __builtin_inff();
    float ulx = inf, uly = inf, ulz = inf, uhx = -inf, uhy = -inf, uhz = -inf;
    auto around = [&](const NodeDev &nd) {
        ulx = fminf(ulx, nd.lox); uly = fminf(uly, nd.loy); ulz = fminf(ulz, nd.loz);
        uhx = fmaxf(uhx, nd.hix); uhy = fmaxf(uhy, nd.hiy); uhz = fmaxf(uhz, nd.hiz);
    };
    for (;;) {
        const bool have = lane < n_front;
        NodeDev nd = {};
        if (have) nd = nodes[my];
        const bool leaf = (nd.info >> 31) != 0u;
        const bool pass = have && shaft_meets(sh, nd);
        const unsigned long long m_pass = ballot(pass), m_exp = ballot(pass && !leaf), m_leaf = m_pass & ~m_exp;
        const uint32_t n_pass = (uint32_t)__popcll(m_pass), n_exp = (uint32_t)__popcll(m_exp), n_leaf = n_pass - n_exp;
        const unsigned long long below = (1ull << lane) - 1ull;
        if (n_out + n_leaf + 2u * n_exp > kMaxCut) {
            if (pass) {
                if (kCutEntriesUsed) out[n_out + (uint32_t)__popcll(m_pass & below)] = CutEntry{my, leaf ? my + 1u : nd.link, nd};
                l_entries[n_out + (uint32_t)__popcll(m_pass & below)] = CutEntry{my, leaf ? my + 1u : nd.link, nd};
                out_stream[n_out + (uint32_t)__popcll(m_pass & below)] = stream_record(my, leaf, nd);
                around(nd);
                const uint32_t size = leaf ? 1u : nd.link - my;
                w += leaf ? 1u + 3u * nd.link : 4u + 6u * (31u - (uint32_t)__clz((int)size));
            }
            n_out += n_pass;
            break;
        }
        if (pass && leaf) {
            if (kCutEntriesUsed) out[n_out + (uint32_t)__popcll(m_leaf & below)] = CutEntry{my, my + 1u, nd};
            l_entries[n_out + (uint32_t)__popcll(m_leaf & below)] = CutEntry{my, my + 1u, nd};
            out_stream[n_out + (uint32_t)__popcll(m_leaf & below)] = nd;
            around(nd);
            w += 1u + 3u * nd.link;
        }
        n_out += n_leaf;
        if (n_exp == 0u) break;
        if (pass && !leaf) {
            const uint32_t k = (uint32_t)__popcll(m_exp & below);
            l_front[2u * k] = my + 1u;
            l_front[2u * k + 1u] = nd.info;
        }
        __builtin_amdgcn_fence(__ATOMIC_RELEASE, "wavefront");
        __builtin_amdgcn_wave_barrier();
        n_front = 2u * n_exp;
        my = l_front[lane];
        __builtin_amdgcn_fence(__ATOMIC_ACQUIRE, "wavefront");
        __builtin_amdgcn_wave_barrier();
    }
    weight = wave_sum(w);
    if (n_out >= 2u) {
        NodeDev all;
        all.lox = wave_min(ulx); all.loy = wave_min(uly); all.loz = wave_min(ulz);
        all.hix = wave_max(uhx); all.hiy = wave_max(uhy); all.hiz = wave_max(uhz);
        all.link = 0u; all.info = 0u;
        if (lane == 0) out_stream[kMaxCut] = all;
    }
    return n_out;
}

constexpr uint32_t kHistShardsLog = 8u, kHistShards = 1u << kHistShardsLog;
constexpr uint32_t kOrderHist = kCostBuckets;
constexpr uint32_t kOrderCursor = kHistShards * kCostBuckets;
constexpr uint32_t kOrderSetWords = kOrderCursor + kCostBuckets;
__host__ __device__ inline StreamWorkspace counting_set(StreamWorkspace W, uint32_t set)
{
    W.buckets += set * kOrderSetWords;
    return W;
}

template <bool COUNT, bool FAST, bool SPHERES, bool WHOLE>
__global__ void __launch_bounds__(64 * kProbeWaves, RTX_PROBE_WAVES_PER_SIMD) probe_kernel(DeviceScene S, TileSpec ts, uint32_t tiles_x, uint32_t n_tiles,
                                                   uint32_t r, StreamWorkspace W, uint8_t *__restrict__ out,
                                                   uint32_t *__restrict__ queue, unsigned long long *__restrict__ counters)
{
    const NodeRec RTX_CONSTANT *nodes = (const NodeRec RTX_CONSTANT *)S.nodes;
    const TriRec RTX_CONSTANT *tris = (const TriRec RTX_CONSTANT *)S.tris;
    __shared__ uint32_t l_front_all[kProbeWaves][128];
    __shared__ CutEntry l_entries_all[kProbeWaves][kMaxCut];
#if RTX_ABLATION
    __shared__ __align__(16) uint32_t l_j1_block[kProbeWaves][kJ1BlockWords];
#endif
    const uint32_t lane = threadIdx.x & 63u;
    const uint32_t wave_in_group = __builtin_amdgcn_readfirstlane(threadIdx.x >> 6);
    uint32_t *const l_front = l_front_all[wave_in_group];
    static_assert(kProbeWaves == 1u, "the XCD mapping assumes one tile per workgroup");
    const uint32_t k = blockIdx.x >> 3;
    const uint32_t tile_id = ((((k >> 6) << 3) + (blockIdx.x & 7u)) << 6) + (k & 63u);
    if (tile_id >= n_tiles) return;
    uint32_t px, py, ly, tile_x, tile_y;
    tile_xy(tile_id, tiles_x, true, tile_x, tile_y);
    const bool in_frame = tile_pixel(S, ts, tile_x, tile_y, lane, px, py, ly);
    WaveCounters wc;
    float dx, dy, dz;
    primary_ray(S, in_frame, px, py, r, dx, dy, dz);
    LaneRay pr = make_ray(in_frame, S.eye[0], S.eye[1], S.eye[2], dx, dy, dz);
    ProbePhaseClock phases;
    phases.mark(0);
#if RTX_ABLATION
    const bool ok = (S.j1_mode == 2u || S.j1_mode == 3u)
        ? j1_closest_hit_blocks<COUNT>(S.j1_mode, S.tris, S.shade, S.n_prims, pr, wc, lane, l_j1_block[wave_in_group])
        : closest_hit<COUNT, FAST, SPHERES>((const NodeRec RTX_CONSTANT *)S.primary_nodes, tris, S.shade, S.n_nodes, pr, wc, S.n_global);
#else
    const bool ok = closest_hit<COUNT, FAST, SPHERES>((const NodeRec RTX_CONSTANT *)S.primary_nodes, tris, S.shade, S.n_nodes, pr, wc, S.n_global);
#endif
    phases.mark(1);
    const bool hit = ok && in_frame && pr.best_idx != kNone;
    const unsigned long long hit_mask = ballot(hit);
    const uint32_t n_hit = (uint32_t)__popcll(hit_mask);
    const uint32_t slot = __popcll(hit_mask & ((1ull << lane) - 1ull));
    const uint32_t first_idx = __builtin_amdgcn_readfirstlane(hit_mask ? __shfl(pr.best_idx, __ffsll((long long)hit_mask) - 1) : 0u);
    const bool one_surface = ballot(hit && pr.best_idx != first_idx) == 0ull;
    uint32_t was_redo = 0u, counted = 0u;
    if (r != 0u) {
        const TileDesc old = W.tiles[tile_id];
        was_redo = old.flags & 2u;
        counted = old.pad;
    }
    uint32_t flags = one_surface ? 1u : 0u;
    if (!ok || was_redo) flags |= 2u;
    if (!ok && !was_redo && lane == 0) {
        queue[kQueueHeader + atomicAdd(&queue[kQueueRedoCount], 1u)] = tile_id;
        if (COUNT && counters) {
            atomicAdd(&counters[5], 1ull);
            if (counted) atomicAdd(&counters[0], 0ull - (unsigned long long)counted);
        }
    }
    float hx = 0.0f, hy = 0.0f, hz = 0.0f;
    const bool compact = one_surface && n_hit != 0u && (!SPHERES || S.shade[first_idx].kind == 0u);
    if (compact) flags |= kTileCompactHits;
    if (hit) {
        const ShadeRec sh = S.shade[pr.best_idx];
        HitRec h;
        h.p[0] = hx = S.eye[0] + pr.best_t * dx;
        h.p[1] = hy = S.eye[1] + pr.best_t * dy;
        h.p[2] = hz = S.eye[2] + pr.best_t * dz;
        hit_normal<SPHERES>(sh, h.p[0], h.p[1], h.p[2], h.n[0], h.n[1], h.n[2]);
        h.rgb[0] = sh.rgb[0]; h.rgb[1] = sh.rgb[1]; h.rgb[2] = sh.rgb[2];
        h.pad[0] = h.pad[1] = h.pad[2] = 0.0f;
        if (compact) {
            float *words = reinterpret_cast<float *>(W.hits + (size_t)tile_id * 64u);
            words[3u * slot] = h.p[0]; words[3u * slot + 1u] = h.p[1]; words[3u * slot + 2u] = h.p[2];
            if (slot == 0u) {
                words[192] = h.n[0]; words[193] = h.n[1]; words[194] = h.n[2];
                words[195] = h.rgb[0]; words[196] = h.rgb[1]; words[197] = h.rgb[2];
            }
        } else {
            W.hits[(size_t)tile_id * 64u + slot] = h;
        }
    }
    if (n_hit != 0u) W.pix_slot[(size_t)tile_id * 64u + lane] = hit ? slot : kNone;
    unsigned long long cost = 0;
    uint32_t n_cut = 0u;
    const uint32_t n_chunks = (n_hit * S.nb_light + 63u) / 64u;
    if (n_hit != 0u && S.nb_light != 0u && !(flags & 2u)) {
        const float inf = __builtin_inff();
        const float olx = wave_min(hit ? hx : inf), ohx = wave_max(hit ? hx : -inf);
        const float oly = wave_min(hit ? hy : inf), ohy = wave_max(hit ? hy : -inf);
        const float olz = wave_min(hit ? hz : inf), ohz = wave_max(hit ? hz : -inf);
        const float *lb = S.light_boxes + 6u * r;
        Shaft sh;
        sh.lower = 0u; sh.upper = 0u;
        shaft_constraint(sh, 0u, ohx, lb[3] - ohx, S.shaft_delta);
        shaft_constraint(sh, 1u, olx, lb[0] - olx, S.shaft_delta);
        shaft_constraint(sh, 2u, ohy, lb[4] - ohy, S.shaft_delta);
        shaft_constraint(sh, 3u, oly, lb[1] - oly, S.shaft_delta);
        shaft_constraint(sh, 4u, ohz, lb[5] - ohz, S.shaft_delta);
        shaft_constraint(sh, 5u, olz, lb[2] - olz, S.shaft_delta);
        uint32_t weight = 0u;
        const uint32_t root = S.n_global != 0u ? 2u : 0u;
        if (!WHOLE && root < S.n_nodes) {
            NodeDev *cut_stream = reinterpret_cast<NodeDev *>(reinterpret_cast<char *>(W.cut) + cut_stream_offset(n_tiles));
            n_cut = shaft_cut_binary(reinterpret_cast<const NodeDev *>(S.nodes), root, sh, W.cut + (size_t)tile_id * kMaxCut,
                                     cut_stream + (size_t)tile_id * kCutStreamRecords, l_front, l_entries_all[wave_in_group], lane, weight);
            if (n_cut != 0u && (flags & 1u)) {
                __builtin_amdgcn_fence(__ATOMIC_RELEASE, "wavefront");
                __builtin_amdgcn_wave_barrier();
                __builtin_amdgcn_fence(__ATOMIC_ACQUIRE, "wavefront");
                const uint32_t walked_weight = RTX_PROBE_VISIT_SCALE *
                    probe_cut_walk<FAST, SPHERES>(nodes, tris, S.shade, reinterpret_cast<const uint32_t *>(l_entries_all[wave_in_group]), n_cut,
                                                  S.n_global, S.light_points + 3u * (r * S.nb_light), hit, hx, hy, hz);
                weight = weight / 2u + walked_weight;
            }
        } else if (WHOLE && root < S.n_nodes) {
            n_cut = 0u;
            const float *lp = S.light_points + 3u * (r * S.nb_light);
            const float vx = lp[0] - hx, vy = lp[1] - hy, vz = lp[2] - hz;
            float dist_light, sx, sy, sz;
// ... 50 lines not shown
```

ray-tracer-rust_amd/csrc/scene_prep.cpp:

```cpp
#include "scene_prep.h"

#include <algorithm>
#include <cfloat>
#include <cmath>
#include <cstdlib>
#include <cstring>
#include <limits>
#include <numeric>

namespace rtx {

namespace {

struct V3 { float x, y, z; };

inline V3 load3(const float *p) { return V3{p[0], p[1], p[2]}; }
inline void store3(float *p, V3 a) { p[0] = a.x; p[1] = a.y; p[2] = a.z; }
inline V3 operator-(V3 a, V3 b) { return V3{a.x - b.x, a.y - b.y, a.z - b.z}; }

inline float dot3(V3 a, V3 b)
{
    float acc = 0.0f;
    acc = acc + a.x * b.x;
    acc = acc + a.y * b.y;
// ... 701 lines not shown
            global_leaf = !std::getenv("RTX_NO_GLOBAL_LEAF");
#endif
            s.n_global = 0;
            Box all;
            all.reset();
            for (const Prim &p : prims) all.grow(p.lo, p.hi);
            const double scene_area = all.half_area();
            if (scene_area > 0 && global_leaf) {
                auto is_global = [&](const Prim &p) {
                    Box b;
                    std::memcpy(b.lo, p.lo, 12);
                    std::memcpy(b.hi, p.hi, 12);
                    return p.kind == 0u && b.half_area() >= 0.5 * scene_area;
                };
                const size_t n = static_cast<size_t>(std::count_if(prims.begin(), prims.end(), is_global));
                if (n >= 1 && n <= kMaxGlobalPrims) {
                    std::stable_partition(prims.begin(), prims.end(), is_global);
                    s.n_global = static_cast<uint32_t>(n);
                }
            }
            float light_c[3] = {0.0f, 0.0f, 0.0f};
            bool light_ok = d.nb_light_sample != 0u;
            if (light_ok) {
                double acc[3] = {0, 0, 0};
                for (uint32_t i = 0; i < d.nb_light_sample; ++i)
                    for (int k = 0; k < 3; ++k) acc[k] += s.light_points[3 * static_cast<size_t>(i) + k];
                for (int k = 0; k < 3; ++k) {
                    light_c[k] = static_cast<float>(acc[k] / d.nb_light_sample);
                    light_ok = light_ok && std::isfinite(light_c[k]);
                }
            }
            {
                TreeBuilder tb(prims, s.nodes, leaf_max, box_cost, 64u, light_ok ? light_c : nullptr);
                if (s.n_global) {
                    Box g;
                    g.reset();
                    for (uint32_t i = 0; i < s.n_global; ++i) g.grow(prims[i].lo, prims[i].hi);
                    NodeRec leaf;
                    std::memcpy(leaf.bmin, g.lo, 12);
                    std::memcpy(leaf.bmax, g.hi, 12);
                    leaf.info = kLeafFlag | 0u;
                    leaf.link = s.n_global;
                    if (s.n_global < n_prims) {
                        NodeRec root;
                        std::memcpy(root.bmin, all.lo, 12);
                        std::memcpy(root.bmax, all.hi, 12);
                        root.info = 0;
                        root.link = 0;
                        s.nodes.push_back(root);
                        s.nodes.push_back(leaf);
                        tb.build(s.n_global, n_prims, 1);
                        s.nodes[0].link = static_cast<uint32_t>(s.nodes.size());
                    } else {
                        s.nodes.push_back(leaf);
                    }
                    s.n_leaves = tb.leaves + 1;
                    s.max_leaf_tris = tb.max_leaf;
                    s.depth = tb.depth + 1;
                } else {
                    tb.build(0, n_prims, 0);
                    s.n_leaves = tb.leaves;
                    s.max_leaf_tris = tb.max_leaf;
                    s.depth = tb.depth;
                }
            }
            finish_tree();
            s.primary_nodes.clear();
            if (s.n_global < n_prims)
                stream_nearest_first(s.nodes, s.n_global != 0u ? 2u : 0u, d.eye, s.primary_nodes);
        }
        s.tris.resize(n_prims);
        std::vector<uint32_t> pos_of(n_prims);
        for (uint32_t i = 0; i < n_prims; ++i) {
            s.tris[i] = recs[prims[i].idx];
            pos_of[prims[i].idx] = i;
        }
        s.global_planes.assign(s.n_global, TriRec{});
        for (uint32_t i = 0; i < s.n_global; ++i) global_plane_statement(s.tris[i], &s.global_planes[i]);
        for (NodeRec &nd : s.ref_nodes)
            if (nd.info & kLeafFlag) {
                const uint32_t prim = nd.info & kLeafIndexMask;
                nd.info = kLeafFlag | (s.shade[prim].kind ? kSphereFlag : 0u) | pos_of[prim];
            }
    } catch (const std::bad_alloc &) {
        return RTX_ERR_OOM;
    }
    return RTX_OK;
}


void pose_tables(const PreparedScene &s, PoseTables &out)
{
    const size_t n_nodes = s.nodes.size(), n_prims = s.shade.size();
    out.ranges.assign(2u * n_nodes, 0u);
    for (size_t i = n_nodes; i-- > 0;) {
        const NodeRec &n = s.nodes[i];
        uint32_t first, end;
        if (n.info & kLeafFlag) {
            first = n.info & kLeafIndexMask;
            end = first + n.link;
        } else {
            const size_t a = i + 1u, b = n.info;
            first = std::min(out.ranges[2u * a], out.ranges[2u * b]);
            end = std::max(out.ranges[2u * a] + out.ranges[2u * a + 1u], out.ranges[2u * b] + out.ranges[2u * b + 1u]);
        }
        out.ranges[2u * i] = first;
        out.ranges[2u * i + 1u] = end - first;
    }
    out.tri_of.assign(n_prims, kPoseNoTriangle);
    uint32_t next = 0;
    for (size_t i = 0; i < n_prims; ++i)
        if (s.shade[i].kind == 0u) out.tri_of[i] = next++;
    out.order.clear();
    out.order.reserve(n_nodes);
    for (uint32_t i = 0; i < n_nodes; ++i)
        if (out.ranges[2u * i + 1u] > kPoseLaneMax) out.order.push_back(i);
    out.n_long = static_cast<uint32_t>(out.order.size());
    for (uint32_t i = 0; i < n_nodes; ++i)
        if (out.ranges[2u * i + 1u] <= kPoseLaneMax) out.order.push_back(i);
}

bool pose_in_range(const PreparedScene &s, const float *pose)
{
    const size_t n = 9u * static_cast<size_t>(s.n_tris - s.n_spheres);
    for (size_t k = 0; k < n; ++k)
        if (!(std::fabs(pose[k]) <= s.scene_magnitude)) return false;
    return true;
}

void posed_records(const PreparedScene &s, const PoseTables &t, const float *pose, const uint32_t *rank, TriRec *tris,
                   ShadeRec *shade, NodeRec *nodes)
{
    const size_t n_prims = s.tris.size();
    std::vector<TriRec> own;
    if (!tris) {
        own.resize(n_prims);
        tris = own.data();
    }
    for (size_t j = 0; j < n_prims; ++j) {
        TriRec r = s.tris[j];
        ShadeRec sh = s.shade[r.idx];
        if (sh.kind == 0u) {
            const float *v = pose + 9u * static_cast<size_t>(t.tri_of[r.idx]);
            std::memcpy(r.v0, v, 12);
            triangle_statement(v, v + 3, v + 6, r.e1, r.e2, sh.normal, r.bmin, r.bmax);
        }
        sh.rank = rank ? rank[r.idx] : r.idx;
        tris[j] = r;
        if (shade) shade[r.idx] = sh;
    }
    if (!nodes) return;
    const float inf = std::numeric_limits<float>::infinity();
    for (size_t i = 0; i < s.nodes.size(); ++i) {
        NodeRec n = s.nodes[i];
        const uint32_t first = t.ranges[2u * i], count = t.ranges[2u * i + 1u];
        for (int k = 0; k < 3; ++k) {
            float lo = inf, hi = -inf;
            for (uint32_t j = first; j < first + count; ++j) {
                lo = fminf(lo, tris[j].bmin[k]);
                hi = fmaxf(hi, tris[j].bmax[k]);
            }
            n.bmin[k] = lo - s.cull_delta;
            n.bmax[k] = hi + s.cull_delta;
        }
        nodes[i] = n;
    }
}

int posed_ref_tree(const PreparedScene &s, const PoseTables &t, const float *pose, std::vector<uint32_t> &rank,
                   std::vector<NodeRec> &stream)
// ... 170 lines not shown
```

ray-tracer-rust_amd/csrc/scene_prep.h:

```cpp
#pragma once

#include <cmath>
#include <cstdint>
#include <vector>

#include "../../include/rtx.h"

#if defined(__HIP__)
#define RTX_HOST_DEVICE __host__ __device__
#else
#define RTX_HOST_DEVICE
#endif

namespace rtx {

RTX_HOST_DEVICE inline void light_sample_point(const float v0[3], const float v1[3], const float v2[3], float u, float v,
                                               float out[3])
{
    const float su = sqrtf(u);
    const float sv = sqrtf(v);
    const float w0 = 1.0f - su;
    const float w1 = su * (1.0f - sv);
    const float w2 = v * su;
    for (int k = 0; k < 3; ++k)
// ... 53 lines not shown
                         v[i].bmin[2] - inflate, v[i].bmax[2] + inflate, v[i].link, v[i].info};
    return out;
}
constexpr uint32_t kLeafFlag = 0x80000000u;
constexpr uint32_t kSphereFlag = 0x40000000u;
constexpr uint32_t kLeafIndexMask = 0x3FFFFFFFu;

struct TriRec {
    float    v0[3];
    float    e1[3];
    float    e2[3];
    float    bmin[3];
    float    bmax[3];
    uint32_t idx;
};
static_assert(sizeof(TriRec) == 64, "TriRec must be 64 bytes");

RTX_HOST_DEVICE inline float f32_successor(float x)
{
    if (!(x < __builtin_inff())) return x;
    uint32_t bits;
    __builtin_memcpy(&bits, &x, 4);
    ++bits;
    __builtin_memcpy(&x, &bits, 4);
    return x;
}
RTX_HOST_DEVICE inline void global_plane_statement(const TriRec &t, TriRec *out)
{
    TriRec g = {};
    const double e1[3] = {t.e1[0], t.e1[1], t.e1[2]}, e2[3] = {t.e2[0], t.e2[1], t.e2[2]};
    double sum_w = 0.0;
    bool fine = true;
    for (int a = 0; a < 3; ++a) {
        const int b = (a + 1) % 3, c = (a + 2) % 3;
        const double n = e1[b] * e2[c] - e1[c] * e2[b];
        const double w = fabs(e1[b] * e2[c]) + fabs(e1[c] * e2[b]);
        g.v0[a] = t.v0[a];
        g.e1[a] = static_cast<float>(n);
        g.e2[a] = f32_successor(static_cast<float>(w));
        fine = fine && w < 0x1p100;
        sum_w += static_cast<double>(g.e2[a]);
    }
    const double kd = 0x1p-19 * 2.0 * sum_w + 0x1p-100;
    g.bmin[0] = fine ? f32_successor(static_cast<float>(kd)) : __builtin_inff();
    g.idx = t.idx;
    *out = g;
}

struct ShadeRec {
    float    normal[3];
    uint32_t rank;
    float    rgb[3];
    uint32_t kind;
};
static_assert(sizeof(ShadeRec) == 32, "ShadeRec must be 32 bytes");

struct PreparedScene {
    uint32_t width = 0, height = 0;
    float eye[3], cam_u[3], cam_v[3], cam_w[3];
    float distance = 0;
    uint32_t nb_ray = 1, nb_light_sample = 0;
    uint32_t n_tris = 0;
    uint32_t n_spheres = 0;
    uint32_t n_samples = 0;
    std::vector<NodeRec>  nodes;
    std::vector<NodeRec>  primary_nodes;
    std::vector<NodeRec>  ref_nodes;
    std::vector<TriRec>   tris;
    std::vector<ShadeRec> shade;
    std::vector<float>    samples;
    float light_v[9];
    std::vector<float>    light_points;
    std::vector<float>    light_tour;
    std::vector<uint32_t> light_order;
    float gamma_thr[256];
    uint32_t n_leaves = 0, max_leaf_tris = 0, depth = 0;
    float cull_delta = 0.0f;
    std::vector<float>    light_boxes;
    float shaft_delta = 0.0f;
    float scene_magnitude = 0.0f;
    uint32_t leaf_max = 4;
    uint32_t n_global = 0;
    std::vector<TriRec>   global_planes;
};
constexpr uint32_t kMaxGlobalPrims = 8u;
constexpr uint64_t kMaxPrimitives = 1ull << 26;

#ifndef RTX_LIGHT_BATCH
#define RTX_LIGHT_BATCH 128
#endif
constexpr uint32_t kMaxLightBatch = RTX_LIGHT_BATCH;

void light_tour_order(const float *points, uint32_t n, uint32_t *order);

void light_tour_order_f32(const float *points, uint32_t n, uint32_t *order);
void light_boxes_of(const float *points, uint32_t nb_ray, uint32_t nb_light, float *out);
float shaft_delta_of(float scene_magnitude, const float *light_boxes, size_t n);

int prepare_scene(const RtxSceneDesc &desc, PreparedScene &out);

void stream_nearest_first(const std::vector<NodeRec> &nodes, uint32_t root, const float *point, std::vector<NodeRec> &out);

void camera_new(const float eye[3], const float look_at[3], const float up[3],
                float u[3], float v[3], float w[3]);
void triangle_derive(const float v0[3], const float v1[3], const float v2[3],
                     float e1[3], float e2[3], float normal[3], float bmin[3], float bmax[3]);
void light_sample(const float v0[3], const float v1[3], const float v2[3], float u, float v, float out[3]);
void light_points_of(const float tri[9], const float *samples, uint32_t n_samples, uint32_t nb_ray, uint32_t nb_light,
                     float *out);
uint8_t gamma_quantise(float linear);
int  build_gamma_thresholds(float thr[256]);
int  ref_leaf_rank(uint32_t n_tris, const float *v0v1v2, uint32_t *out_rank);
int  ref_tree_build(uint32_t n_tris, const float *v0v1v2, uint32_t *out_rank, std::vector<NodeRec> *out_stream);
int  ref_tree_build_boxes(uint32_t n, const float *lo_hi, uint32_t *out_rank, std::vector<NodeRec> *out_stream);
constexpr uint32_t kRefTreeAutoMax = 50000u;

constexpr uint32_t kPoseLaneMax = 32u;
constexpr uint32_t kPoseBlock = 256u;
constexpr uint32_t kPoseNoTriangle = 0xFFFFFFFFu;
struct PoseTables {
    std::vector<uint32_t> ranges;
    std::vector<uint32_t> tri_of;
    std::vector<uint32_t> order;
    uint32_t n_long = 0;
};
void pose_tables(const PreparedScene &s, PoseTables &out);
bool pose_in_range(const PreparedScene &s, const float *pose);
void posed_records(const PreparedScene &s, const PoseTables &t, const float *pose, const uint32_t *rank, TriRec *tris,
                   ShadeRec *shade, NodeRec *nodes);
int posed_ref_tree(const PreparedScene &s, const PoseTables &t, const float *pose, std::vector<uint32_t> &rank,
                   std::vector<NodeRec> &stream);


constexpr uint32_t kRebuildCellBits = 21u;
constexpr uint32_t kRebuildCellMax = (1u << kRebuildCellBits) - 1u;
inline float rebuild_key_scale(float bound) { return static_cast<float>(2097152.0 / (2.0 * static_cast<double>(bound))); }
RTX_HOST_DEVICE inline uint64_t rebuild_key_statement(const float bmin[3], const float bmax[3], bool sphere, float bound,
                                                      float scale)
{
    uint64_t key = sphere ? 1ull << 63 : 0ull;
    for (int k = 0; k < 3; ++k) {
        const float c = 0.5f * (bmin[k] + bmax[k]);
        const float f = (c + bound) * scale;
        uint32_t q = 0u;
        if (f >= 2097151.0f) q = kRebuildCellMax;
        else if (f >= 0.0f) q = static_cast<uint32_t>(f);
        uint64_t x = q;
        x = (x | x << 32) & 0x1F00000000FFFFull;
        x = (x | x << 16) & 0x1F0000FF0000FFull;
        x = (x | x << 8) & 0x100F00F00F00F00Full;
        x = (x | x << 4) & 0x10C30C30C30C30C3ull;
        x = (x | x << 2) & 0x1249249249249249ull;
        key |= x << (2 - k);
    }
    return key;
}
struct RebuildTables {
    std::vector<NodeRec>  nodes;
    std::vector<uint32_t> ranges;
    std::vector<uint32_t> order;
    uint32_t n_long = 0;
    uint32_t n_tree_tris = 0, n_tree_spheres = 0;
};
void rebuild_tables(const PreparedScene &s, RebuildTables &out);
void rebuilt_records(const PreparedScene &s, const PoseTables &t, const RebuildTables &b, const float *pose,
                     const uint32_t *rank, uint64_t *keys, uint32_t *perm, TriRec *tris, ShadeRec *shade, NodeRec *nodes);
int rebuilt_ref_tree(const PreparedScene &s, const PoseTables &t, const float *pose, const uint32_t *perm,
// ... 4 lines not shown
```

ray-tracer-rust_amd/rtx.py:

```python
import ctypes as C
import os

import numpy as np

_HERE = os.path.dirname(os.path.abspath(__file__))
LIB_PATH = os.environ.get("RTX_PY_LIB") or os.path.join(
    _HERE, "librtx_ablation.so" if os.environ.get("RTX_PY_ABLATION") == "1" else "librtx.so")

if not os.path.exists(LIB_PATH):
    raise ImportError(
        "%s is not built. Build it with: python -c 'import __graft_entry__ as g; g.build()' "
        "or make -C ray-tracer-rust_amd/csrc [ablation]" % LIB_PATH)

_lib = C.CDLL(LIB_PATH)

OK, ERR_BAD_ARG, ERR_NO_DEVICE, ERR_HIP, ERR_OOM, ERR_UNSUPPORTED, ERR_INTERNAL, ERR_IO = 0, -1, -2, -3, -4, -5, -6, -7
ACCEL_BVH, ACCEL_BRUTE = 0, 1
REFTREE_AUTO, REFTREE_ALWAYS, REFTREE_NEVER = 0, 1, 2

NB_RAY, NB_LIGHT_SAMPLE, NB_RAND_SAMPLE = 1, 100, 2000000
DEFAULT_EYE = (0.0, 100.0, 200.0)
DEFAULT_LOOK_AT = (0.0, 0.0, -100000.0)
DEFAULT_UP = (0.0, 1.0, 0.0)
DEFAULT_DISTANCE = 288.0
# ... 80 lines not shown


_SIGS = {
    "rtx_abi_version": (C.c_int, []),
    "rtx_device_count": (C.c_int, []),
    "rtx_scene_create": (C.c_int, [C.POINTER(SceneDesc), C.POINTER(C.c_void_p)]),
    "rtx_scene_destroy": (None, [C.c_void_p]),
    "rtx_scene_info": (C.c_int, [C.c_void_p, C.POINTER(SceneInfo)]),
    "rtx_scene_upload": (C.c_int, [C.c_void_p, C.c_int]),
    "rtx_render_rows": (C.c_int, [C.c_void_p, C.c_int, C.c_uint32, C.c_uint32, C.c_void_p, C.POINTER(Stats)]),
    "rtx_render_frame": (C.c_int, [C.c_void_p, C.POINTER(C.c_int), C.c_int, C.c_uint32, C.c_void_p, C.POINTER(Stats)]),
    "rtx_render_tiles_device": (C.c_int, [C.c_void_p, C.c_int, C.c_uint32, C.c_uint32, C.c_uint32, C.c_void_p,
                                          C.c_size_t, C.c_void_p, C.c_void_p]),
    "rtx_tiles_rows": (C.c_uint32, [C.c_void_p, C.c_uint32, C.c_uint32, C.c_uint32]),
    "rtx_tiles_bytes": (C.c_size_t, [C.c_void_p, C.c_uint32, C.c_uint32, C.c_uint32]),
    "rtx_trace_rays": (C.c_int, [C.c_void_p, C.c_int, C.c_uint32, f32p, f32p, C.c_uint32, C.POINTER(RayHit), C.POINTER(Stats)]),
    "rtx_occluded_rays": (C.c_int, [C.c_void_p, C.c_int, C.c_uint32, f32p, f32p, C.c_uint32, u8p, C.POINTER(Stats)]),
    "rtx_trace_rays_device": (C.c_int, [C.c_void_p, C.c_int, C.c_uint32, C.c_void_p, C.c_void_p, C.c_uint32, C.c_void_p, C.c_void_p]),
    "rtx_occluded_rays_device": (C.c_int, [C.c_void_p, C.c_int, C.c_uint32, C.c_void_p, C.c_void_p, C.c_uint32, C.c_void_p, C.c_void_p]),
    "rtx_shade_rays": (C.c_int, [C.c_void_p, C.c_int, C.c_uint32, f32p, f32p, C.c_uint32, C.POINTER(PixelShade),
                                 C.POINTER(RayHit), C.POINTER(Stats)]),
    "rtx_shade_rays_device": (C.c_int, [C.c_void_p, C.c_int, C.c_uint32, C.c_void_p, C.c_void_p, C.c_uint32, C.c_void_p,
                                        C.c_void_p, C.c_void_p]),
    "rtx_scene_view": (C.c_int, [C.c_void_p, C.POINTER(RtxView)]),
    "rtx_render_view": (C.c_int, [C.c_void_p, C.c_int, C.POINTER(RtxView), C.c_void_p, C.POINTER(PixelShade), C.POINTER(RayHit),
                                  C.POINTER(Stats)]),
    "rtx_render_view_device": (C.c_int, [C.c_void_p, C.c_int, C.POINTER(RtxView), C.c_void_p, C.c_void_p, C.c_void_p, C.c_void_p]),
    "rtx_render_view_rows": (C.c_int, [C.c_void_p, C.c_int, C.POINTER(RtxView), C.c_void_p, C.POINTER(Stats)]),
    "rtx_render_view_rows_device": (C.c_int, [C.c_void_p, C.c_int, C.POINTER(RtxView), C.c_void_p, C.c_size_t, C.c_void_p,
                                              C.c_void_p]),
    "rtx_scene_aimed_nodes": (C.c_int, [C.c_void_p, f32p, u32p]),
    "rtx_debug_aimed_nodes": (C.c_int, [C.c_void_p, C.c_int, f32p, u32p]),
    "rtx_scene_light": (C.c_int, [C.c_void_p, C.POINTER(RtxLight)]),
    "rtx_scene_light_points_for": (C.c_int, [C.c_void_p, C.POINTER(RtxLight), f32p]),
    "rtx_debug_light_points": (C.c_int, [C.c_void_p, C.c_int, C.POINTER(RtxLight), f32p]),
    "rtx_render_view_rows_lit": (C.c_int, [C.c_void_p, C.c_int, C.POINTER(RtxView), C.POINTER(RtxLight), C.c_void_p,
                                           C.POINTER(Stats)]),
    "rtx_render_view_rows_lit_device": (C.c_int, [C.c_void_p, C.c_int, C.POINTER(RtxView), C.POINTER(RtxLight), C.c_void_p,
                                                  C.c_size_t, C.c_void_p, C.c_void_p]),
    "rtx_scene_light_walk_for": (C.c_int, [C.c_void_p, C.POINTER(RtxLight), u32p, f32p, f32p]),
    "rtx_debug_light_walk": (C.c_int, [C.c_void_p, C.c_int, C.POINTER(RtxLight), f32p, f32p]),
    "rtx_render_view_lit": (C.c_int, [C.c_void_p, C.c_int, C.POINTER(RtxView), C.POINTER(RtxLight), C.c_void_p,
                                      C.POINTER(PixelShade), C.POINTER(RayHit), C.POINTER(Stats)]),
    "rtx_render_view_lit_device": (C.c_int, [C.c_void_p, C.c_int, C.POINTER(RtxView), C.POINTER(RtxLight), C.c_void_p, C.c_void_p,
                                             C.c_void_p, C.c_void_p]),
    "rtx_shade_rays_lit": (C.c_int, [C.c_void_p, C.c_int, C.c_uint32, f32p, f32p, C.c_uint32, C.POINTER(RtxLight),
                                     C.POINTER(PixelShade), C.POINTER(RayHit), C.POINTER(Stats)]),
    "rtx_shade_rays_lit_device": (C.c_int, [C.c_void_p, C.c_int, C.c_uint32, C.c_void_p, C.c_void_p, C.c_uint32,
                                            C.POINTER(RtxLight), C.c_void_p, C.c_void_p, C.c_void_p]),
    "rtx_scene_pose_bound": (C.c_int, [C.c_void_p, f32p]),
    "rtx_scene_pose": (C.c_int, [C.c_void_p, C.c_int, f32p, u32p, C.c_uint32, C.POINTER(Stats)]),
    "rtx_scene_pose_device": (C.c_int, [C.c_void_p, C.c_int, C.c_void_p, C.c_void_p, C.c_void_p]),
    "rtx_scene_posed_records": (C.c_int, [C.c_void_p, f32p, u32p, u32p, u32p, u32p]),
    "rtx_debug_pose": (C.c_int, [C.c_void_p, C.c_int, u32p, u32p, u32p]),
    "rtx_trace_rays_posed": (C.c_int, [C.c_void_p, C.c_int, C.c_uint32, f32p, f32p, C.c_uint32, C.POINTER(RayHit), C.POINTER(Stats)]),
    "rtx_occluded_rays_posed": (C.c_int, [C.c_void_p, C.c_int, C.c_uint32, f32p, f32p, C.c_uint32, u8p, C.POINTER(Stats)]),
    "rtx_trace_rays_posed_device": (C.c_int, [C.c_void_p, C.c_int, C.c_uint32, C.c_void_p, C.c_void_p, C.c_uint32, C.c_void_p,
                                              C.c_void_p]),
    "rtx_occluded_rays_posed_device": (C.c_int, [C.c_void_p, C.c_int, C.c_uint32, C.c_void_p, C.c_void_p, C.c_uint32, C.c_void_p,
                                                 C.c_void_p]),
    "rtx_shade_rays_posed": (C.c_int, [C.c_void_p, C.c_int, C.c_uint32, f32p, f32p, C.c_uint32, C.POINTER(RtxLight),
                                       C.POINTER(PixelShade), C.POINTER(RayHit), C.POINTER(Stats)]),
    "rtx_shade_rays_posed_device": (C.c_int, [C.c_void_p, C.c_int, C.c_uint32, C.c_void_p, C.c_void_p, C.c_uint32,
                                              C.POINTER(RtxLight), C.c_void_p, C.c_void_p, C.c_void_p]),
    "rtx_render_view_posed": (C.c_int, [C.c_void_p, C.c_int, C.POINTER(RtxView), C.POINTER(RtxLight), C.c_void_p,
                                        C.POINTER(PixelShade), C.POINTER(RayHit), C.POINTER(Stats)]),
    "rtx_render_view_posed_device": (C.c_int, [C.c_void_p, C.c_int, C.POINTER(RtxView), C.POINTER(RtxLight), C.c_void_p, C.c_void_p,
                                               C.c_void_p, C.c_void_p]),
    "rtx_render_view_rows_posed": (C.c_int, [C.c_void_p, C.c_int, C.POINTER(RtxView), C.POINTER(RtxLight), C.c_void_p,
                                             C.POINTER(Stats)]),
    "rtx_render_view_rows_posed_device": (C.c_int, [C.c_void_p, C.c_int, C.POINTER(RtxView), C.POINTER(RtxLight), C.c_void_p,
                                                    C.c_size_t, C.c_void_p, C.c_void_p]),
    "rtx_scene_posed_pipeline_records": (C.c_int, [C.c_void_p, f32p, f32p, u32p, u32p]),
    "rtx_debug_pose_pipeline": (C.c_int, [C.c_void_p, C.c_int, f32p, u32p, u32p]),
    "rtx_scene_pose_rebuilt": (C.c_int, [C.c_void_p, C.c_int, f32p, u32p, C.c_uint32, C.POINTER(Stats)]),
    "rtx_scene_pose_rebuilt_device": (C.c_int, [C.c_void_p, C.c_int, C.c_void_p, C.c_void_p, C.c_void_p]),
    "rtx_scene_rebuilt_counts": (C.c_int, [C.c_void_p, u32p]),
    "rtx_scene_rebuilt_records": (C.c_int, [C.c_void_p, f32p, u32p, C.POINTER(C.c_uint64), u32p, u32p, u32p, u32p]),
    "rtx_scene_rebuilt_aimed": (C.c_int, [C.c_void_p, f32p, f32p, u32p]),
    "rtx_debug_pose_rebuilt": (C.c_int, [C.c_void_p, C.c_int, f32p, u32p, u32p, u32p, u32p, u32p]),
    "rtx_debug_wave_profile": (C.c_int, [C.c_void_p, C.c_int, C.c_uint32, C.c_uint32, u64p, C.c_size_t, u32p, u32p]),
    "rtx_launch_timings": (C.c_int, [C.c_void_p, C.c_int, C.c_int, f32p, f32p]),
    "rtx_debug_tile_descs": (C.c_int, [C.c_void_p, C.c_int, u32p, C.c_size_t]),
    "rtx_strerror": (C.c_char_p, [C.c_int]),
    "rtx_last_hip_error": (C.c_int, []),
    "rtx_scene_light_points": (C.c_int, [C.c_void_p, f32p]),
    "rtx_scene_light_order": (C.c_int, [C.c_void_p, u32p]),
    "rtx_scene_gamma_thresholds": (C.c_int, [C.c_void_p, f32p]),
    "rtx_scene_normals": (C.c_int, [C.c_void_p, f32p]),
    "rtx_scene_nodes": (C.c_int, [C.c_void_p, u32p, u32p]),
    "rtx_scene_primary_nodes": (C.c_int, [C.c_void_p, u32p, u32p]),
    "rtx_scene_ref_nodes": (C.c_int, [C.c_void_p, u32p]),
    "rtxh_camera_new": (None, [f32p] * 6),
    "rtxh_import_obj": (C.c_int, [C.c_char_p, C.POINTER(f32p)]),
    "rtxh_import_obj_ex": (C.c_int, [C.c_char_p, C.c_uint32, C.POINTER(f32p), C.POINTER(f32p)]),
    "rtxh_free": (None, [C.c_void_p]),
    "rtxh_ref_leaf_rank": (C.c_int, [C.c_uint32, f32p, u32p]),
    "rtxh_gen_samples": (None, [C.c_uint64, C.c_uint32, f32p]),
    "rtxh_write_png": (C.c_int, [C.c_char_p, C.c_uint32, C.c_uint32, C.c_void_p]),
    "rtxh_synthetic_mesh": (C.c_int, [C.c_uint64, C.c_uint32, f32p]),
    "rtxh_scatter_tiles": (C.c_int, [C.c_void_p, C.c_uint32, C.c_uint32, C.c_void_p, C.c_uint32, C.c_uint32, C.c_uint32]),
}
for _name, (_res, _args) in _SIGS.items():
    _fn = getattr(_lib, _name)
    _fn.restype = _res
    _fn.argtypes = _args


class RtxError(RuntimeError):
    def __init__(self, code, where=""):
        self.code = code
        msg = _lib.rtx_strerror(code).decode()
        if code == ERR_HIP:
            msg += " (hipError %d)" % _lib.rtx_last_hip_error()
        super().__init__("%s: %s [%d]" % (where, msg, code))


def _check(code, where):
    if code != OK:
        raise RtxError(code, where)


def _fp(a):
    return a.ctypes.data_as(f32p)


def _f3(x):
    return np.ascontiguousarray(np.asarray(x, dtype=np.float32).reshape(3))


def abi_version():
    return _lib.rtx_abi_version()


def device_count():
    return _lib.rtx_device_count()


def camera_new(eye, look_at, up):
    u, v, w = (np.zeros(3, np.float32) for _ in range(3))
    _lib.rtxh_camera_new(_fp(_f3(eye)), _fp(_f3(look_at)), _fp(_f3(up)), _fp(u), _fp(v), _fp(w))
    return u, v, w


def import_obj(path):
    p = f32p()
    n = _lib.rtxh_import_obj(os.fsencode(path), C.byref(p))
    if n < 0:
        raise RtxError(n, "rtxh_import_obj(%s)" % path)
    arr = np.ctypeslib.as_array(p, shape=(max(n, 1), 9))[:n].copy() if n else np.zeros((0, 9), np.float32)
    _lib.rtxh_free(p)
    return arr


OBJ_SLASHES, OBJ_RELATIVE, OBJ_POLYGONS, OBJ_MATERIALS, OBJ_ALL = 1, 2, 4, 8, 15


def import_obj_ex(path, flags=OBJ_ALL):
    t, c = f32p(), f32p()
    n = _lib.rtxh_import_obj_ex(os.fsencode(path), flags, C.byref(t), C.byref(c))
    if n < 0:
        raise RtxError(n, "rtxh_import_obj_ex(%s)" % path)
    tris = np.ctypeslib.as_array(t, shape=(max(n, 1), 9))[:n].copy() if n else np.zeros((0, 9), np.float32)
    rgb = np.ctypeslib.as_array(c, shape=(max(n, 1), 3))[:n].copy() if n else np.zeros((0, 3), np.float32)
    _lib.rtxh_free(t)
    _lib.rtxh_free(c)
# ... 142 lines not shown
            _check(_lib.rtx_scene_light_order(self._h, out.ctypes.data_as(u32p)), "rtx_scene_light_order")
        return out

    def gamma_thresholds(self):
        out = np.zeros(256, np.float32)
        _check(_lib.rtx_scene_gamma_thresholds(self._h, _fp(out)), "rtx_scene_gamma_thresholds")
        return out

    def normals(self):
        out = np.zeros((self.n_prims, 3), np.float32)
        _check(_lib.rtx_scene_normals(self._h, _fp(out)), "rtx_scene_normals")
        return out

    def nodes(self):
        i = self.info()
        nd = np.zeros((i["n_nodes"], 8), np.uint32)
        order = np.zeros(i["n_tris"], np.uint32)
        _check(_lib.rtx_scene_nodes(self._h, nd.ctypes.data_as(u32p), order.ctypes.data_as(u32p)), "rtx_scene_nodes")
        return nd, order

    def primary_nodes(self):
        nd = np.zeros((self.info()["n_nodes"], 8), np.uint32)
        own = C.c_uint32(0)
        _check(_lib.rtx_scene_primary_nodes(self._h, nd.ctypes.data_as(u32p), C.cast(C.byref(own), u32p)), "rtx_scene_primary_nodes")
        return nd, bool(own.value)

    def ref_nodes(self):
        nd = np.zeros((self.info()["n_ref_nodes"], 8), np.uint32)
        if len(nd):
            _check(_lib.rtx_scene_ref_nodes(self._h, nd.ctypes.data_as(u32p)), "rtx_scene_ref_nodes")
        return nd

    def upload(self, device=0):
        _check(_lib.rtx_scene_upload(self._h, device), "rtx_scene_upload")

    def render_rows(self, row0=0, nrows=None, device=0, stats=False, out_ptr=None):
        if nrows is None:
            nrows = self.height - row0
        out = None if out_ptr else np.zeros((nrows, self.width, 3), np.uint8)
        st = Stats()
        _check(_lib.rtx_render_rows(self._h, device, row0, nrows, C.c_void_p(out_ptr) if out_ptr else out.ctypes.data,
                                    C.byref(st) if stats else None), "rtx_render_rows")
        if out_ptr:
            return st.asdict() if stats else None
        return (out, st.asdict()) if stats else out

    def render_frame(self, devices=(0,), tile_rows=8, stats=False):
        out = np.zeros((self.height, self.width, 3), np.uint8)
        devs = (C.c_int * len(devices))(*devices)
        st = Stats()
        _check(_lib.rtx_render_frame(self._h, devs, len(devices), tile_rows, out.ctypes.data,
                                     C.byref(st) if stats else None), "rtx_render_frame")
        return (out, st.asdict()) if stats else out

    def wave_profile(self, row0=0, nrows=None, device=0):
        if nrows is None:
            nrows = self.height - row0
        tx, ty = C.c_uint32(), C.c_uint32()
        _check(_lib.rtx_debug_wave_profile(self._h, device, row0, nrows, None, 0, C.byref(tx), C.byref(ty)),
               "rtx_debug_wave_profile")
        out = np.zeros((ty.value, tx.value, 8), np.uint64)
        _check(_lib.rtx_debug_wave_profile(self._h, device, row0, nrows, out.ctypes.data_as(u64p), tx.value * ty.value,
                                           C.byref(tx), C.byref(ty)), "rtx_debug_wave_profile")
        return out

    def launch_timings(self, device=0, max_launches=64):
        a = np.zeros(max_launches, np.float32)
        b = np.zeros(max_launches, np.float32)
        n = _lib.rtx_launch_timings(self._h, device, max_launches, _fp(a), _fp(b))
        if n < 0:
            raise RtxError(n, "rtx_launch_timings")
        return a[:n], b[:n]

    def tile_descs(self, device=0):
        n = _lib.rtx_debug_tile_descs(self._h, device, None, 0)
        if n < 0:
            raise RtxError(n, "rtx_debug_tile_descs")
        out = np.zeros((n, 4), np.uint32)
        m = _lib.rtx_debug_tile_descs(self._h, device, out.ctypes.data_as(u32p), n)
        if m < 0:
            raise RtxError(m, "rtx_debug_tile_descs")
        return out[:m]

    def tiles_rows(self, first_tile, tile_stride, tile_rows):
        return _lib.rtx_tiles_rows(self._h, first_tile, tile_stride, tile_rows)

    def tiles_bytes(self, first_tile, tile_stride, tile_rows):
        return _lib.rtx_tiles_bytes(self._h, first_tile, tile_stride, tile_rows)

    def render_tiles_device(self, device, first_tile, tile_stride, tile_rows, d_out_ptr, d_out_bytes,
                            stream=None, d_counters_ptr=None):
        _check(_lib.rtx_render_tiles_device(self._h, device, first_tile, tile_stride, tile_rows,
                                            C.c_void_p(d_out_ptr), d_out_bytes,
                                            C.c_void_p(stream) if stream else None,
                                            C.c_void_p(d_counters_ptr) if d_counters_ptr else None),
               "rtx_render_tiles_device")

    @staticmethod
    def _ray_flags(keep_order, force_regroup):
        return (RAYS_KEEP_ORDER if keep_order else 0) | (RAYS_FORCE_REGROUP if force_regroup else 0)

    @staticmethod
    def _ray_arrays(first, second):
        a = np.ascontiguousarray(first, dtype=np.float32).reshape(-1, 3)
        b = np.ascontiguousarray(second, dtype=np.float32).reshape(-1, 3)
        if len(a) != len(b):
            raise ValueError("the two ray arrays disagree in length")
        return a, b

    def trace_rays(self, origins, directions, device=0, keep_order=False, stats=False, force_regroup=False, posed=False):
        o, d = self._ray_arrays(origins, directions)
        out = np.zeros(len(o), RAY_HIT_DTYPE)
        st = Stats()
        fn = _lib.rtx_trace_rays_posed if posed else _lib.rtx_trace_rays
        _check(fn(self._h, device, len(o), _fp(o), _fp(d), self._ray_flags(keep_order, force_regroup),
                  out.ctypes.data_as(C.POINTER(RayHit)), C.byref(st) if stats else None), "rtx_trace_rays")
        return (out, st.asdict()) if stats else out

    def occluded_rays(self, origins, targets, device=0, keep_order=False, stats=False, force_regroup=False, posed=False):
        o, t = self._ray_arrays(origins, targets)
        out = np.zeros(len(o), np.uint8)
        st = Stats()
        fn = _lib.rtx_occluded_rays_posed if posed else _lib.rtx_occluded_rays
        _check(fn(self._h, device, len(o), _fp(o), _fp(t), self._ray_flags(keep_order, force_regroup),
                  out.ctypes.data_as(u8p), C.byref(st) if stats else None), "rtx_occluded_rays")
        return (out, st.asdict()) if stats else out

    def trace_rays_device(self, device, n_rays, d_origins_ptr, d_directions_ptr, d_hits_ptr, stream=None,
                          keep_order=False, force_regroup=False, posed=False):
        fn = _lib.rtx_trace_rays_posed_device if posed else _lib.rtx_trace_rays_device
        _check(fn(self._h, device, n_rays, C.c_void_p(d_origins_ptr), C.c_void_p(d_directions_ptr),
                  self._ray_flags(keep_order, force_regroup), C.c_void_p(d_hits_ptr),
                  C.c_void_p(stream) if stream else None), "rtx_trace_rays_device")

    def occluded_rays_device(self, device, n_rays, d_origins_ptr, d_targets_ptr, d_occluded_ptr, stream=None,
                             keep_order=False, force_regroup=False, posed=False):
        fn = _lib.rtx_occluded_rays_posed_device if posed else _lib.rtx_occluded_rays_device
        _check(fn(self._h, device, n_rays, C.c_void_p(d_origins_ptr), C.c_void_p(d_targets_ptr),
                  self._ray_flags(keep_order, force_regroup), C.c_void_p(d_occluded_ptr),
                  C.c_void_p(stream) if stream else None), "rtx_occluded_rays_device")

    @staticmethod
    def _lit_or_posed(stem, form, head, tail, light, posed):
        if posed:
            name, mid = stem + "_posed" + form, (C.byref(light) if light is not None else None,)
        elif light is None:
            name, mid = stem + form, ()
        else:
            name, mid = stem + "_lit" + form, (C.byref(light),)
        _check(getattr(_lib, name)(*head, *mid, *tail), name)

    def shade_rays(self, origins, directions, device=0, keep_order=False, stats=False, force_regroup=False,
                   want_hits=False, light=None, posed=False):
        o, d = self._ray_arrays(origins, directions)
        if len(o) % self.nb_ray:
            raise ValueError("a pixel is nb_ray = %d consecutive rays" % self.nb_ray)
        n = len(o) // self.nb_ray
        out = np.zeros(n, PIXEL_SHADE_DTYPE)
        hits = np.zeros(len(o), RAY_HIT_DTYPE) if want_hits else None
        st = Stats()
        tail = (out.ctypes.data_as(C.POINTER(PixelShade)), hits.ctypes.data_as(C.POINTER(RayHit)) if want_hits else None,
                C.byref(st) if stats else None)
        head = (self._h, device, n, _fp(o), _fp(d), self._ray_flags(keep_order, force_regroup))
        self._lit_or_posed("rtx_shade_rays", "", head, tail, light, posed)
        res = (out,) + ((hits,) if want_hits else ()) + ((st.asdict(),) if stats else ())
        return res if len(res) > 1 else out
# ... 249 lines not shown
```

Measured before the change: 138,100.

## Predict expensive probe tiles on host and split them across multiple waves

During scene prep the host estimates a per-tile traversal weight by testing each 8x8 tile's view frustum against the BVH node stream, and records the heaviest tiles (above a threshold, capped). These long tiles are uploaded with a bitmask, and the probe kernel launches a variant with four waves per block, giving the listed long tiles extra parallelism in front of the regular tiles. The aim is to cut the tail latency of the probe pass caused by a few very deep tiles. This adds host prep cost, a larger grid, and a heuristic that can be wrong for other camera poses.

```diff
diff --git a/include/rtx.h b/include/rtx.h
--- a/include/rtx.h
+++ b/include/rtx.h
@@ -221,6 +221,13 @@
 int rtx_launch_timings(RtxScene *scene, int device, int max_launches, float *schedule_ms, float *shade_ms);
 
 int rtx_debug_tile_descs(RtxScene *scene, int device, uint32_t *out, size_t max_tiles);
+int rtx_debug_probe_records(RtxScene *scene, int device, uint32_t *out_hits, uint32_t *out_pix_slots, size_t max_tiles);
+
+int rtx_scene_probe_long(const RtxScene *scene, uint32_t *out_tiles, uint32_t *out_weights, size_t max_entries,
+                         uint32_t *out_threshold);
+int rtx_scene_probe_tile(const RtxScene *scene, uint32_t tile_x, uint32_t tile_y, uint8_t *out_met ,
+                         uint32_t *out_weight);
+int rtx_debug_probe_split(RtxScene *scene, uint32_t mode);
 
 const char *rtx_strerror(int err);
 int rtx_last_hip_error(void);
diff --git a/integration/rtx_ffi.rs b/integration/rtx_ffi.rs
--- a/integration/rtx_ffi.rs
+++ b/integration/rtx_ffi.rs
@@ -235,6 +235,13 @@
                                 out_boxes: *mut f32) -> c_int;
     pub fn rtx_launch_timings(scene: *mut RtxScene, device: c_int, max_launches: c_int, schedule_ms: *mut f32,
                               shade_ms: *mut f32) -> c_int;
+    pub fn rtx_scene_probe_long(scene: *const RtxScene, out_tiles: *mut u32, out_weights: *mut u32, max_entries: usize,
+                                out_threshold: *mut u32) -> c_int;
+    pub fn rtx_scene_probe_tile(scene: *const RtxScene, tile_x: u32, tile_y: u32, out_met: *mut u8,
+                                out_weight: *mut u32) -> c_int;
+    pub fn rtx_debug_probe_split(scene: *mut RtxScene, mode: u32) -> c_int;
+    pub fn rtx_debug_probe_records(scene: *mut RtxScene, device: c_int, out_hits: *mut u32, out_pix_slots: *mut u32,
+                                   max_tiles: usize) -> c_int;
     pub fn rtx_strerror(err: c_int) -> *const c_char;
     pub fn rtx_last_hip_error() -> c_int;
     pub fn rtxh_scatter_tiles(frame: *mut u8, height: u32, width: u32, packed: *const u8, first_tile: u32,
diff --git a/ray-tracer-rust_amd/csrc/rtx_api.cpp b/ray-tracer-rust_amd/csrc/rtx_api.cpp
--- a/ray-tracer-rust_amd/csrc/rtx_api.cpp
+++ b/ray-tracer-rust_amd/csrc/rtx_api.cpp
@@ -8,6 +8,7 @@
 #include <cstdlib>
 #include <cstring>
 #include <initializer_list>
+#include <atomic>
 #include <map>
 #include <memory>
 #include <mutex>
@@ -154,6 +155,8 @@
     Event q_sorted;
     DeviceGeometry geo;
     DeviceBuffer primary_nodes, samples, lights, light_tour, thr, light_boxes;
+    DeviceBuffer long_words, long_all;
+    uint32_t n_long_all = 0;
     DeviceBuffer d_out, d_counters;
     DeviceBuffer d_redo;
     bool launch_words_ready = false;
@@ -234,6 +237,7 @@
     rtx::RebuildTables rebuild_tables;
     bool rebuild_tables_made = false;
     std::map<int, DeviceSlot> dev;
+    std::atomic<uint32_t> split_mode{0u}, last_long{0u};
 };
 
 namespace {
@@ -303,6 +307,11 @@
     if ((rc = upload_vec(st.light_tour, p.light_tour)) != RTX_OK) return rc;
     if (!p.global_planes.empty() && (rc = upload_vec(g.planes, p.global_planes)) != RTX_OK) return rc;
     if ((rc = upload_vec(st.light_boxes, p.light_boxes)) != RTX_OK) return rc;
+    if (!p.long_tiles.empty()) {
+        std::vector<uint32_t> words(p.long_tiles);
+        words.insert(words.end(), p.long_bits.begin(), p.long_bits.end());
+        if ((rc = upload_vec(st.long_words, words)) != RTX_OK) return rc;
+    }
     if ((rc = st.thr.reserve(sizeof(p.gamma_thr))) != RTX_OK) return rc;
     RTX_HIP(hipMemcpy(st.thr.as<void>(), p.gamma_thr, sizeof(p.gamma_thr), hipMemcpyHostToDevice));
     if ((rc = st.d_counters.reserve(rtx::kNumCounters * sizeof(unsigned long long))) != RTX_OK) return rc;
@@ -474,7 +483,8 @@
 
 template <class Before>
 int render_launch(DeviceState &st, const rtx::DeviceScene &S, const rtx::TileSpec &ts, uint8_t *d_out,
-                  unsigned long long *d_counters, unsigned long long *d_wave_prof, hipStream_t stream, Before before)
+                  unsigned long long *d_counters, unsigned long long *d_wave_prof, hipStream_t stream, Before before,
+                  const rtx::ProbeSplit &split = rtx::ProbeSplit{nullptr, 0u, 0u, 0u})
 {
     int rc;
     const size_t redo_cap = st.d_redo.capacity(), buckets_cap = st.ws.buckets.capacity();
@@ -492,7 +502,7 @@
     }
     if (ts.local_rows) st.launch_words_ready = false;
     RTX_HIP(rtx::launch_trace_shade(S, ts, d_out, st.d_redo.as<uint32_t>(), use_ws ? &ws : nullptr, d_counters, d_wave_prof,
-                                    kernel_variant(), stream, d_wave_prof ? nullptr : phases, st.words_launches, st.words_passes));
+                                    kernel_variant(), stream, d_wave_prof ? nullptr : phases, st.words_launches, st.words_passes, split));
     if (two_pass) {
         st.launch_words_ready = true;
         ++st.words_launches;
@@ -502,14 +512,43 @@
     return RTX_OK;
 }
 
+int probe_split_of(RtxScene *scene, DeviceState &st, const rtx::DeviceScene &S, const rtx::TileSpec &ts, rtx::ProbeSplit *out)
+{
+    *out = rtx::ProbeSplit{nullptr, 0u, 0u, 0u};
+    scene->last_long = 0u;
+    const uint32_t mode = scene->split_mode;
+    if (mode == 1u || !rtx::probe_split_applies(S, ts)) return RTX_OK;
+    if (mode == 2u) {
+        if (!st.n_long_all) {
+            const uint32_t n = ((S.width + 7u) / 8u) * ((S.height + 7u) / 8u);
+            std::vector<uint32_t> words(n + (n + 31u) / 32u, 0xFFFFFFFFu);
+            for (uint32_t t = 0; t < n; ++t) words[t] = t;
+            RTX_TRY(upload_vec(st.long_all, words));
+            st.n_long_all = n;
+        }
+        const uint32_t tx = (S.width + 7u) / 8u, ty = (S.height + 7u) / 8u;
+        if (tx - 1u <= 0xFFFFu && ty - 1u <= 0xFFFFu)
+            *out = rtx::ProbeSplit{st.long_all.as<const uint32_t>(), st.n_long_all, (tx - 1u) << 16, (ty - 1u) << 16};
+    } else if (!scene->prep.long_tiles.empty()) {
+        const std::vector<uint32_t> &tiles = scene->prep.long_tiles;
+        rtx::ProbeSplit listed{st.long_words.as<const uint32_t>(), static_cast<uint32_t>(tiles.size()), 0u, 0u};
+        if (rtx::probe_split_ranges(tiles.data(), listed.n_long, (S.width + 7u) / 8u, &listed)) *out = listed;
+    }
+    scene->last_long = out->n_long;
+    return RTX_OK;
+}
+
 int launch_on(RtxScene *scene, DeviceSlot &slot, const rtx::TileSpec &ts, const Timed &timed)
 {
     RTX_TRY(ensure_uploaded(scene, slot));
     DeviceState &st = *slot.st;
     const size_t bytes = static_cast<size_t>(ts.local_rows) * scene->prep.width * 3u;
     RTX_TRY(st.d_out.reserve(bytes ? bytes : 16));
-    RTX_TRY(render_launch(st, device_scene(scene, st, st.geo), ts, st.d_out.as<uint8_t>(), timed.counters(st), nullptr, st.stream,
-                          [&] { return timed.begin(st); }));
+    const rtx::DeviceScene S = device_scene(scene, st, st.geo);
+    rtx::ProbeSplit split;
+    RTX_TRY(probe_split_of(scene, st, S, ts, &split));
+    RTX_TRY(render_launch(st, S, ts, st.d_out.as<uint8_t>(), timed.counters(st), nullptr, st.stream,
+                          [&] { return timed.begin(st); }, split));
     return timed.end(st);
 }
 
@@ -1073,6 +1112,7 @@
     S.distance = v.distance;
     S.primary_nodes = aimed_stream(scene, g);
     const rtx::TileSpec ts{v.y0, v.ny, v.ny, v.ny};
+    scene->last_long = 0u;
     return render_launch(st, S, ts, d_out, d_counters, nullptr, stream, [&]() -> int {
         RTX_TRY(before());
         RTX_TRY(aim_at(scene, g, v.eye, stream));
@@ -1458,9 +1498,12 @@
     Entry e(scene, device, Entry::kUploaded);
     if (e.rc != RTX_OK) return e.rc;
     const rtx::TileSpec ts{first_tile * tile_rows, tile_rows, tile_stride * tile_rows, rows};
-    return render_launch(e.state(), device_scene(scene, e.state(), e.state().geo), ts, static_cast<uint8_t *>(d_out_rgb),
+    const rtx::DeviceScene S = device_scene(scene, e.state(), e.state().geo);
+    rtx::ProbeSplit split;
+    RTX_TRY(probe_split_of(scene, e.state(), S, ts, &split));
+    return render_launch(e.state(), S, ts, static_cast<uint8_t *>(d_out_rgb),
                          reinterpret_cast<unsigned long long *>(d_counters), nullptr, static_cast<hipStream_t>(stream),
-                         [] { return static_cast<int>(RTX_OK); });
+                         [] { return static_cast<int>(RTX_OK); }, split);
 }
 
 int rtx_trace_rays(RtxScene *scene, int device, uint32_t n_rays, const float *origins, const float *directions,
@@ -1969,6 +2012,51 @@
     return static_cast<int>(n);
 }
 
+int rtx_debug_probe_records(RtxScene *scene, int device, uint32_t *out_hits, uint32_t *out_pix_slots, size_t max_tiles)
+{
+    if (!scene) return RTX_ERR_BAD_ARG;
+    Entry e(scene, device, Entry::kLocked);
+    if (e.rc != RTX_OK) return e.rc;
+    const DeviceState &st = e.state();
+    if (!out_hits && !out_pix_slots) return static_cast<int>(st.last_tiles);
+    const int rc = e.make_current();
+    if (rc != RTX_OK) return rc;
+    const size_t n = st.last_tiles < max_tiles ? st.last_tiles : max_tiles;
+    RTX_HIP(hipDeviceSynchronize());
+    if (n && out_hits) RTX_HIP(hipMemcpy(out_hits, st.ws.hits.as<void>(), n * 64u * sizeof(rtx::HitRec), hipMemcpyDeviceToHost));
+    if (n && out_pix_slots) RTX_HIP(hipMemcpy(out_pix_slots, st.ws.pix_slot.as<void>(), n * 64u * sizeof(uint32_t), hipMemcpyDeviceToHost));
+    return static_cast<int>(n);
+}
+
+int rtx_debug_probe_split(RtxScene *scene, uint32_t mode)
+{
+    if (!scene || mode > 2u) return RTX_ERR_BAD_ARG;
+    scene->split_mode = mode;
+    return static_cast<int>(scene->last_long.load());
+}
+
+int rtx_scene_probe_long(const RtxScene *scene, uint32_t *out_tiles, uint32_t *out_weights, size_t max_entries, uint32_t *out_threshold)
+{
+    if (!scene) return RTX_ERR_BAD_ARG;
+    const rtx::PreparedScene &p = scene->prep;
+    const size_t n = p.long_tiles.size() < max_entries ? p.long_tiles.size() : max_entries;
+    if (out_tiles && n) std::memcpy(out_tiles, p.long_tiles.data(), n * sizeof(uint32_t));
+    if (out_weights && n) std::memcpy(out_weights, p.long_weights.data(), n * sizeof(uint32_t));
+    if (out_threshold) *out_threshold = rtx::kProbeLongWeight;
+    return static_cast<int>(out_tiles || out_weights ? n : p.long_tiles.size());
+}
+
+int rtx_scene_probe_tile(const RtxScene *scene, uint32_t tile_x, uint32_t tile_y, uint8_t *out_met, uint32_t *out_weight)
+{
+    if (!scene || !out_weight) return RTX_ERR_BAD_ARG;
+    const rtx::PreparedScene &p = scene->prep;
+    if (tile_x >= (p.width + 7u) / 8u || tile_y >= (p.height + 7u) / 8u) return RTX_ERR_BAD_ARG;
+    if (out_met) std::memset(out_met, 0, p.nodes.size());
+    bool valid = false;
+    *out_weight = rtx::probe_tile_weight(p, tile_x, tile_y, out_met, &valid);
+    return valid ? 1 : 0;
+}
+
 int rtx_launch_timings(RtxScene *scene, int device, int max_launches, float *schedule_ms, float *shade_ms)
 {
     if (!scene || max_launches < 0 || !schedule_ms || !shade_ms) return RTX_ERR_BAD_ARG;
diff --git a/ray-tracer-rust_amd/csrc/rtx_device.h b/ray-tracer-rust_amd/csrc/rtx_device.h
--- a/ray-tracer-rust_amd/csrc/rtx_device.h
+++ b/ray-tracer-rust_amd/csrc/rtx_device.h
@@ -37,6 +37,26 @@
     uint32_t j1_mode;
 };
 constexpr uint32_t kCutMaxNodes = 1u << 16;
+static_assert(kCutMaxNodes == kProbeSplitMaxNodes, "a scene predicts long tiles exactly when it cuts per tile");
+
+struct ProbeSplit {
+    const uint32_t *words;
+    uint32_t n_long;
+    uint32_t x_range, y_range;
+};
+inline bool probe_split_ranges(const uint32_t *tiles, uint32_t n, uint32_t tiles_x, ProbeSplit *out)
+{
+    uint32_t x0 = 0xFFFFu, x1 = 0u, y0 = 0xFFFFu, y1 = 0u;
+    for (uint32_t i = 0; i < n; ++i) {
+        const uint32_t y = tiles[i] / tiles_x, x = tiles[i] - y * tiles_x;
+        if (x > 0xFFFFu || y > 0xFFFFu) return false;
+        x0 = x < x0 ? x : x0; x1 = x > x1 ? x : x1;
+        y0 = y < y0 ? y : y0; y1 = y > y1 ? y : y1;
+    }
+    out->x_range = x0 | x1 << 16;
+    out->y_range = y0 | y1 << 16;
+    return n != 0u;
+}
 
 struct TileSpec {
     uint32_t first_row;
@@ -107,7 +127,19 @@
 hipError_t launch_trace_shade(const DeviceScene &S, const TileSpec &ts, uint8_t *d_out, uint32_t *d_redo,
                               const StreamWorkspace *ws, unsigned long long *d_counters,
                               unsigned long long *d_wave_prof, uint32_t variant, hipStream_t stream,
-                              hipEvent_t *phase_events = nullptr, uint32_t launch_no = 0u, uint32_t pass_no = 0u);
+                              hipEvent_t *phase_events = nullptr, uint32_t launch_no = 0u, uint32_t pass_no = 0u,
+                              const ProbeSplit &split = ProbeSplit{nullptr, 0u, 0u, 0u});
+inline bool tiles_frame_aligned(const TileSpec &ts)
+{
+    return ts.first_row % 8u == 0u && ts.tile_stride_rows != 0u && ts.tile_rows != 0u &&
+           ((ts.tile_rows % 8u == 0u && ts.tile_stride_rows % 8u == 0u) || ts.local_rows <= ts.tile_rows);
+}
+constexpr uint32_t kProbeSplitMaxTiles = 65536u;
+inline bool probe_split_applies(const DeviceScene &S, const TileSpec &ts)
+{
+    const uint64_t tiles = static_cast<uint64_t>((S.width + 7u) / 8u) * ((ts.local_rows + 7u) / 8u);
+    return S.n_nodes <= S.cut_max_nodes && ts.local_rows != 0u && tiles_frame_aligned(ts) && tiles <= kProbeSplitMaxTiles;
+}
 hipError_t zero_launch_words(uint32_t *d_redo, const StreamWorkspace &ws, hipStream_t stream);
 
 }
diff --git a/ray-tracer-rust_amd/csrc/rtx_kernel.hip b/ray-tracer-rust_amd/csrc/rtx_kernel.hip
--- a/ray-tracer-rust_amd/csrc/rtx_kernel.hip
+++ b/ray-tracer-rust_amd/csrc/rtx_kernel.hip
@@ -101,14 +101,13 @@
 template <bool COUNT, bool FAST, bool SPHERES>
 hipError_t launch_probe(const DeviceScene &S, const TileSpec &ts, uint8_t *d_out, uint32_t *d_redo,
                         const StreamWorkspace &W, unsigned long long *d_counters, hipStream_t stream, hipEvent_t *ev,
-                        uint32_t launch_no, uint32_t pass_no)
+                        uint32_t launch_no, uint32_t pass_no, const ProbeSplit &split_in)
 {
 #ifndef RTX_SHADE_NW
 #define RTX_SHADE_NW 8
 #endif
     constexpr int NW = RTX_SHADE_NW;
     const bool whole = S.n_nodes > S.cut_max_nodes;
-    const auto probe = whole ? probe_kernel<COUNT, FAST, SPHERES, true> : probe_kernel<COUNT, FAST, SPHERES, false>;
     const auto shade = whole ? shade_tiles_kernel<COUNT, FAST, NW, SPHERES, true> : shade_tiles_kernel<COUNT, FAST, NW, SPHERES, false>;
     const uint32_t batch = S.nb_light < kMaxLightBatch ? (S.nb_light ? S.nb_light : 1u) : kMaxLightBatch;
 #if RTX_ABLATION
@@ -118,6 +117,11 @@
 #endif
     const uint32_t tiles_x = (S.width + 7u) / 8u, tiles_y = (ts.local_rows + 7u) / 8u;
     const uint32_t n_tiles = numbered_tiles(tiles_x, tiles_y);
+    const ProbeSplit split = (split_in.n_long != 0u && split_in.words && probe_split_applies(S, ts)) ? split_in : ProbeSplit{nullptr, 0u, 0u, 0u};
+    const uint32_t probe_waves = split.n_long != 0u ? 4u : 1u;
+    const uint32_t probe_grid = split.n_long != 0u ? ((split.n_long + 7u) & ~7u) + 128u * ((n_tiles + 511u) / 512u) : 512u * ((n_tiles + 511u) / 512u);
+    const auto probe = whole ? probe_kernel<COUNT, FAST, SPHERES, true, 1u>
+                     : split.n_long != 0u ? probe_kernel<COUNT, FAST, SPHERES, false, 4u> : probe_kernel<COUNT, FAST, SPHERES, false, 1u>;
     static thread_local int cached_dev = -1, cached_blocks = 0;
     static thread_local size_t cached_lds = 0;
     static thread_local bool cached_whole = false;
@@ -141,8 +145,8 @@
     for (uint32_t r = 0; r < S.nb_ray; ++r) {
         const uint32_t hist_set = (pass_no + r) & 1u;
         const StreamWorkspace Wp = counting_set(W, hist_set);
-        hipLaunchKernelGGL(probe, dim3(512u * ((n_tiles + 511u) / 512u)), dim3(64 * kProbeWaves), 0, stream,
-                           S, ts, tiles_x, n_tiles, r, Wp, d_out, queue, d_counters);
+        hipLaunchKernelGGL(probe, dim3(probe_grid), dim3(64 * probe_waves), 0, stream,
+                           S, ts, tiles_x, n_tiles, r, Wp, d_out, queue, d_counters, split);
         if (whole) hipLaunchKernelGGL(count_classes_kernel, dim3((n_tiles + 1023u) / 1024u), dim3(1024), 0, stream, n_tiles, Wp);
         hipLaunchKernelGGL(order_tiles_kernel, dim3((n_tiles + 1023u) / 1024u), dim3(1024), 0, stream, n_tiles, W, grid, split_share(),
                            hist_set, whole ? 0u : grid, queue, next_redo_count);
@@ -196,14 +200,14 @@
 static hipError_t launch_dispatch(const DeviceScene &S, const TileSpec &ts, uint8_t *d_out, uint32_t *d_redo,
                                   const StreamWorkspace *ws, unsigned long long *d_counters,
                                   unsigned long long *d_wave_prof, uint32_t variant, hipStream_t stream, hipEvent_t *ev,
-                                  uint32_t launch_no, uint32_t pass_no)
+                                  uint32_t launch_no, uint32_t pass_no, const ProbeSplit &split)
 {
     auto two_pass = [&](auto fast) {
         constexpr bool FAST = decltype(fast)::value;
         const bool count = d_counters != nullptr, spheres = S.n_spheres != 0u;
         const auto launch = count ? (spheres ? launch_probe<true, FAST, true> : launch_probe<true, FAST, false>)
                                   : (spheres ? launch_probe<false, FAST, true> : launch_probe<false, FAST, false>);
-        return launch(S, ts, d_out, d_redo, *ws, d_counters, stream, ev, launch_no, pass_no);
+        return launch(S, ts, d_out, d_redo, *ws, d_counters, stream, ev, launch_no, pass_no, split);
     };
 #if RTX_ABLATION
     if (!((variant & kVariantProbe) && ws && !d_wave_prof))
@@ -218,14 +222,14 @@
 hipError_t launch_trace_shade(const DeviceScene &S, const TileSpec &ts, uint8_t *d_out, uint32_t *d_redo,
                               const StreamWorkspace *ws, unsigned long long *d_counters,
                               unsigned long long *d_wave_prof, uint32_t variant, hipStream_t stream,
-                              hipEvent_t *phase_events, uint32_t launch_no, uint32_t pass_no)
+                              hipEvent_t *phase_events, uint32_t launch_no, uint32_t pass_no, const ProbeSplit &split)
 {
     if (ts.local_rows == 0) return hipSuccess;
     hipError_t e;
     if (phase_events && (e = hipEventRecord(phase_events[0], stream)) != hipSuccess) return e;
     const bool probe = (variant & kVariantProbe) && ws && !d_wave_prof;
     if (phase_events && !probe && (e = hipEventRecord(phase_events[1], stream)) != hipSuccess) return e;
-    e = launch_dispatch(S, ts, d_out, d_redo, ws, d_counters, d_wave_prof, variant, stream, probe ? phase_events : nullptr, launch_no, pass_no);
+    e = launch_dispatch(S, ts, d_out, d_redo, ws, d_counters, d_wave_prof, variant, stream, probe ? phase_events : nullptr, launch_no, pass_no, split);
     if (e != hipSuccess) return e;
     if (phase_events && (e = hipEventRecord(phase_events[2], stream)) != hipSuccess) return e;
     return hipSuccess;
@@ -238,7 +242,7 @@
 #define RTX_SW(x) " " #x "=" RTX_SW_STR(x)
 extern "C" __attribute__((used, visibility("hidden"))) const char rtx_build_switches_text[] = "rtx-build-switches:"
     RTX_SW(RTX_CLAIM_RUN_LOG) RTX_SW(RTX_CUT_DRAW_MIN) RTX_SW(RTX_CUT_UNION_MIN) RTX_SW(RTX_LIGHT_BATCH) RTX_SW(RTX_MAX_CUT)
-    RTX_SW(RTX_PACKED_WAVES_PER_SIMD) RTX_SW(RTX_PROBE_VISIT_SCALE) RTX_SW(RTX_PROBE_WAVES_PER_SIMD)
+    RTX_SW(RTX_PACKED_WAVES_PER_SIMD) RTX_SW(RTX_PROBE_LONG_WEIGHT) RTX_SW(RTX_PROBE_VISIT_SCALE) RTX_SW(RTX_PROBE_WAVES_PER_SIMD)
     RTX_SW(RTX_SHADE_CUT_WAVES_PER_SIMD) RTX_SW(RTX_SHADE_NW) RTX_SW(RTX_SHADE_WAVES_PER_SIMD)
     RTX_SW(RTX_SPLIT_SHARE_PERCENT) RTX_SW(RTX_TILE_PARTS_MAX) RTX_SW(RTX_WAVES_PER_SIMD)
     RTX_SW(RTX_EXPERIMENT_TIMELINE) RTX_SW(RTX_EXPERIMENT_PHASES) RTX_SW(RTX_EXPERIMENT_PROBE_PHASES) RTX_SW(RTX_ABLATION);
diff --git a/ray-tracer-rust_amd/csrc/rtx_pass_schedule.hpp b/ray-tracer-rust_amd/csrc/rtx_pass_schedule.hpp
--- a/ray-tracer-rust_amd/csrc/rtx_pass_schedule.hpp
+++ b/ray-tracer-rust_amd/csrc/rtx_pass_schedule.hpp
@@ -22,7 +22,6 @@
 #define RTX_CUT_DRAW_MIN 1
 #endif
 constexpr bool kCutEntriesUsed = RTX_ABLATION != 0;
-constexpr uint32_t kProbeWaves = 1u;
 #ifndef RTX_PROBE_WAVES_PER_SIMD
 #define RTX_PROBE_WAVES_PER_SIMD 8
 #endif
@@ -187,41 +186,94 @@
     return W;
 }
 
-template <bool COUNT, bool FAST, bool SPHERES, bool WHOLE>
-__global__ void __launch_bounds__(64 * kProbeWaves, RTX_PROBE_WAVES_PER_SIMD) probe_kernel(DeviceScene S, TileSpec ts, uint32_t tiles_x, uint32_t n_tiles,
+template <bool COUNT, bool FAST, bool SPHERES, bool WHOLE, uint32_t WAVES>
+__global__ void __launch_bounds__(64 * WAVES, RTX_PROBE_WAVES_PER_SIMD) probe_kernel(DeviceScene S, TileSpec ts, uint32_t tiles_x, uint32_t n_tiles,
                                                    uint32_t r, StreamWorkspace W, uint8_t *__restrict__ out,
-                                                   uint32_t *__restrict__ queue, unsigned long long *__restrict__ counters)
+                                                   uint32_t *__restrict__ queue, unsigned long long *__restrict__ counters,
+                                                   ProbeSplit split)
 {
     const NodeRec RTX_CONSTANT *nodes = (const NodeRec RTX_CONSTANT *)S.nodes;
     const TriRec RTX_CONSTANT *tris = (const TriRec RTX_CONSTANT *)S.tris;
-    __shared__ uint32_t l_front_all[kProbeWaves][128];
-    __shared__ CutEntry l_entries_all[kProbeWaves][kMaxCut];
+    static_assert(WAVES == 1u || WAVES == 4u, "one tile per workgroup, or four tiles / the four beams of a long tile");
+    constexpr bool kSplits = WAVES == 4u;
+    __shared__ uint32_t l_front_all[WAVES][128];
+    __shared__ CutEntry l_entries_all[WAVES][kMaxCut];
+    __shared__ float l_beam_t[kSplits ? 64 : 1];
+    __shared__ uint32_t l_beam_idx[kSplits ? 64 : 1];
+    __shared__ uint32_t l_beam_ok[WAVES];
 #if RTX_ABLATION
-    __shared__ __align__(16) uint32_t l_j1_block[kProbeWaves][kJ1BlockWords];
+    __shared__ __align__(16) uint32_t l_j1_block[WAVES][kJ1BlockWords];
 #endif
     const uint32_t lane = threadIdx.x & 63u;
     const uint32_t wave_in_group = __builtin_amdgcn_readfirstlane(threadIdx.x >> 6);
     uint32_t *const l_front = l_front_all[wave_in_group];
-    static_assert(kProbeWaves == 1u, "the XCD mapping assumes one tile per workgroup");
-    const uint32_t k = blockIdx.x >> 3;
-    const uint32_t tile_id = ((((k >> 6) << 3) + (blockIdx.x & 7u)) << 6) + (k & 63u);
-    if (tile_id >= n_tiles) return;
-    uint32_t px, py, ly, tile_x, tile_y;
-    tile_xy(tile_id, tiles_x, true, tile_x, tile_y);
+    const uint32_t n_long = kSplits ? split.n_long : 0u, long_groups = (n_long + 7u) & ~7u;
+    const bool long_mode = kSplits && blockIdx.x < n_long;
+    uint32_t tile_id, tile_x, tile_y;
+    if (long_mode) {
+        const uint32_t entry = __builtin_amdgcn_readfirstlane(split.words[blockIdx.x]);
+        const uint32_t fy = entry / tiles_x;
+        tile_x = entry - fy * tiles_x;
+        const uint32_t row = fy * 8u;
+        if (row < ts.first_row) return;
+        const uint32_t band = (row - ts.first_row) / ts.tile_stride_rows, off = (row - ts.first_row) - band * ts.tile_stride_rows;
+        const uint32_t ly0 = band * ts.tile_rows + off;
+        if (off >= ts.tile_rows || ly0 >= ts.local_rows) return;
+        tile_y = ly0 >> 3;
+        tile_id = ((((tile_y >> 3) * ((tiles_x + 7u) >> 3)) + (tile_x >> 3)) << 6) + ((tile_y & 7u) << 3) + (tile_x & 7u);
+        if (tile_id >= n_tiles) return;
+        if (COUNT && wave_in_group != 0u) return;
+    } else if (!kSplits) {
+        const uint32_t k = blockIdx.x >> 3;
+        tile_id = ((((k >> 6) << 3) + (blockIdx.x & 7u)) << 6) + (k & 63u);
+        if (tile_id >= n_tiles) return;
+        tile_xy(tile_id, tiles_x, true, tile_x, tile_y);
+    } else {
+        if (blockIdx.x < long_groups) return;
+        const uint32_t g = blockIdx.x - long_groups, k = g >> 3;
+        tile_id = ((((k >> 4) << 3) + (g & 7u)) << 6) + ((k & 15u) << 2) + wave_in_group;
+        if (tile_id >= n_tiles) return;
+        tile_xy(tile_id, tiles_x, true, tile_x, tile_y);
+        if (n_long != 0u) {
+            const uint32_t ly0 = tile_y * 8u, band = ly0 < ts.tile_rows ? 0u : ly0 / ts.tile_rows;
+            const uint32_t fy = (ts.first_row + band * ts.tile_stride_rows + (ly0 - band * ts.tile_rows)) >> 3;
+            if (tile_x >= (split.x_range & 0xFFFFu) && tile_x <= (split.x_range >> 16) && fy >= (split.y_range & 0xFFFFu) &&
+                fy <= (split.y_range >> 16) && ly0 < ts.local_rows) {
+                const uint32_t t = fy * tiles_x + tile_x;
+                if ((split.words[n_long + (t >> 5)] >> (t & 31u)) & 1u) return;
+            }
+        }
+    }
+    uint32_t px, py, ly;
     const bool in_frame = tile_pixel(S, ts, tile_x, tile_y, lane, px, py, ly);
     WaveCounters wc;
     float dx, dy, dz;
     primary_ray(S, in_frame, px, py, r, dx, dy, dz);
-    LaneRay pr = make_ray(in_frame, S.eye[0], S.eye[1], S.eye[2], dx, dy, dz);
+    const bool beams = long_mode && !COUNT;
+    const bool walks = in_frame && (!beams || (((lane >> 5) << 1) | ((lane >> 2) & 1u)) == wave_in_group);
+    LaneRay pr = make_ray(walks, S.eye[0], S.eye[1], S.eye[2], dx, dy, dz);
     ProbePhaseClock phases;
     phases.mark(0);
+    bool ok = true;
+    if (!beams || ballot(walks) != 0ull) {
 #if RTX_ABLATION
-    const bool ok = (S.j1_mode == 2u || S.j1_mode == 3u)
-        ? j1_closest_hit_blocks<COUNT>(S.j1_mode, S.tris, S.shade, S.n_prims, pr, wc, lane, l_j1_block[wave_in_group])
-        : closest_hit<COUNT, FAST, SPHERES>((const NodeRec RTX_CONSTANT *)S.primary_nodes, tris, S.shade, S.n_nodes, pr, wc, S.n_global);
+        ok = (S.j1_mode == 2u || S.j1_mode == 3u)
+            ? j1_closest_hit_blocks<COUNT>(S.j1_mode, S.tris, S.shade, S.n_prims, pr, wc, lane, l_j1_block[wave_in_group])
+            : closest_hit<COUNT, FAST, SPHERES>((const NodeRec RTX_CONSTANT *)S.primary_nodes, tris, S.shade, S.n_nodes, pr, wc, S.n_global);
 #else
-    const bool ok = closest_hit<COUNT, FAST, SPHERES>((const NodeRec RTX_CONSTANT *)S.primary_nodes, tris, S.shade, S.n_nodes, pr, wc, S.n_global);
-#endif
+        ok = closest_hit<COUNT, FAST, SPHERES>((const NodeRec RTX_CONSTANT *)S.primary_nodes, tris, S.shade, S.n_nodes, pr, wc, S.n_global);
+#endif
+    }
+    if (beams) {
+        if (walks) { l_beam_t[lane] = pr.best_t; l_beam_idx[lane] = pr.best_idx; }
+        else if ((((lane >> 5) << 1) | ((lane >> 2) & 1u)) == wave_in_group) { l_beam_t[lane] = __builtin_inff(); l_beam_idx[lane] = kNone; }
+        if (lane == 0) l_beam_ok[wave_in_group] = ok ? 1u : 0u;
+        __syncthreads();
+        if (wave_in_group != 0u) return;
+        pr.best_t = l_beam_t[lane];
+        pr.best_idx = l_beam_idx[lane];
+        ok = (l_beam_ok[0] & l_beam_ok[1] & l_beam_ok[2] & l_beam_ok[3]) != 0u;
+    }
     phases.mark(1);
     const bool hit = ok && in_frame && pr.best_idx != kNone;
     const unsigned long long hit_mask = ballot(hit);
diff --git a/ray-tracer-rust_amd/csrc/scene_prep.cpp b/ray-tracer-rust_amd/csrc/scene_prep.cpp
--- a/ray-tracer-rust_amd/csrc/scene_prep.cpp
+++ b/ray-tracer-rust_amd/csrc/scene_prep.cpp
@@ -807,10 +807,146 @@
                 const uint32_t prim = nd.info & kLeafIndexMask;
                 nd.info = kLeafFlag | (s.shade[prim].kind ? kSphereFlag : 0u) | pos_of[prim];
             }
+        for (int c = 0; c < 2; ++c) {
+            float lo = d.samples[c], hi = d.samples[c];
+            bool finite = true;
+            for (size_t i = 0; i < d.n_samples; ++i) {
+                const float v = d.samples[2 * i + c];
+                finite = finite && std::isfinite(v);
+                lo = v < lo ? v : lo;
+                hi = v > hi ? v : hi;
+            }
+            s.sample_lo[c] = finite ? lo : std::nanf("");
+            s.sample_hi[c] = finite ? hi : std::nanf("");
+        }
+        predict_long_tiles(s, kProbeLongWeight);
     } catch (const std::bad_alloc &) {
         return RTX_ERR_OOM;
     }
     return RTX_OK;
+}
+
+
+namespace {
+
+struct ProbePredictor {
+    const PreparedScene &s;
+    const std::vector<NodeRec> &stream;
+    std::vector<double> box;
+    uint32_t root = 0;
+    bool usable = false;
+    explicit ProbePredictor(const PreparedScene &scene)
+        : s(scene), stream(scene.primary_nodes.empty() ? scene.nodes : scene.primary_nodes)
+    {
+        root = (s.n_global != 0u && stream.size() > 2u) ? 2u : (s.n_global != 0u ? static_cast<uint32_t>(stream.size()) : 0u);
+        usable = stream.size() <= kProbeSplitMaxNodes && s.width && s.height;
+        for (int c = 0; c < 2; ++c) usable = usable && std::isfinite(s.sample_lo[c]) && std::isfinite(s.sample_hi[c]);
+        if (!usable) return;
+        box.resize(6 * stream.size());
+        for (size_t i = 0; i < stream.size(); ++i)
+            for (int k = 0; k < 3; ++k) {
+                box[6 * i + k] = static_cast<double>(stream[i].bmin[k] - s.cull_delta) - static_cast<double>(s.eye[k]);
+                box[6 * i + 3 + k] = static_cast<double>(stream[i].bmax[k] + s.cull_delta) - static_cast<double>(s.eye[k]);
+            }
+    }
+    bool planes_of(uint32_t tile_x, uint32_t tile_y, double n[4][3]) const
+    {
+        const double lo0 = std::fmin(static_cast<double>(s.sample_lo[0]), 0.0), hi0 = std::fmax(static_cast<double>(s.sample_hi[0]), 1.0);
+        const double lo1 = std::fmin(static_cast<double>(s.sample_lo[1]), 0.0), hi1 = std::fmax(static_cast<double>(s.sample_hi[1]), 1.0);
+        const double a0 = 8.0 * tile_x - 0.5 * s.width + lo0 - 1.0, a1 = 8.0 * tile_x + 7.0 - 0.5 * s.width + hi0 + 1.0;
+        const double b0 = 8.0 * tile_y - 0.5 * s.height + lo1 - 1.0, b1 = 8.0 * tile_y + 7.0 - 0.5 * s.height + hi1 + 1.0;
+        auto dir = [&](double a, double b, double out[3]) {
+            for (int k = 0; k < 3; ++k)
+                out[k] = a * s.cam_u[k] + b * s.cam_v[k] - static_cast<double>(s.distance) * s.cam_w[k];
+        };
+        double c[4][3], mid[3];
+        dir(a0, b0, c[0]); dir(a1, b0, c[1]); dir(a1, b1, c[2]); dir(a0, b1, c[3]);
+        dir(0.5 * (a0 + a1), 0.5 * (b0 + b1), mid);
+        for (int e = 0; e < 4; ++e) {
+            const double *p = c[e], *q = c[(e + 1) % 4];
+            n[e][0] = p[1] * q[2] - p[2] * q[1];
+            n[e][1] = p[2] * q[0] - p[0] * q[2];
+            n[e][2] = p[0] * q[1] - p[1] * q[0];
+            double inside = n[e][0] * mid[0] + n[e][1] * mid[1] + n[e][2] * mid[2];
+            if (inside < 0.0) {
+                for (int k = 0; k < 3; ++k) n[e][k] = -n[e][k];
+                inside = -inside;
+            }
+            if (!(inside > 0.0) || !std::isfinite(inside)) return false;
+        }
+        return true;
+    }
+    bool meets(const double n[4][3], size_t i) const
+    {
+        const double *b = &box[6 * i];
+        for (int e = 0; e < 4; ++e) {
+            double far = 0.0;
+            for (int k = 0; k < 3; ++k) far += n[e][k] * (n[e][k] > 0.0 ? b[3 + k] : b[k]);
+            if (far < 0.0) return false;
+        }
+        return true;
+    }
+    uint32_t weigh(uint32_t tile_x, uint32_t tile_y, uint8_t *met, bool *valid) const
+    {
+        double n[4][3];
+        *valid = usable && planes_of(tile_x, tile_y, n);
+        if (!*valid) return 0u;
+        if (met)
+            for (uint32_t i = 0; i < root && i < stream.size(); ++i) met[i] = 1;
+        uint64_t w = 0;
+        for (size_t i = root; i < stream.size();) {
+            const NodeRec &nd = stream[i];
+            const bool leaf = (nd.info & kLeafFlag) != 0u;
+            const bool pass = meets(n, i);
+            if (pass) {
+                w += leaf ? 1u + 3ull * nd.link : 1u;
+                if (met) met[i] = 1;
+            }
+            i = (leaf || pass) ? i + 1 : (nd.link > i ? nd.link : stream.size());
+        }
+        return w > 0xFFFFFFFFull ? 0xFFFFFFFFu : static_cast<uint32_t>(w);
+    }
+};
+
+}
+
+uint32_t probe_tile_weight(const PreparedScene &s, uint32_t tile_x, uint32_t tile_y, uint8_t *met, bool *valid)
+{
+    const ProbePredictor p(s);
+    return p.weigh(tile_x, tile_y, met, valid);
+}
+
+void predict_long_tiles(PreparedScene &s, uint32_t threshold)
+{
+    s.long_tiles.clear();
+    s.long_weights.clear();
+    s.long_bits.clear();
+    const ProbePredictor p(s);
+    if (!p.usable) return;
+    const uint32_t tiles_x = (s.width + 7u) / 8u, tiles_y = (s.height + 7u) / 8u;
+    const uint64_t n_tiles64 = static_cast<uint64_t>(tiles_x) * tiles_y;
+    if (n_tiles64 > 0x7FFFFFFFull) return;
+    const uint32_t n_tiles = static_cast<uint32_t>(n_tiles64), cap = probe_long_cap(n_tiles);
+    if (cap == 0u) return;
+    std::vector<std::pair<uint32_t, uint32_t>> found;
+    for (uint32_t ty = 0; ty < tiles_y; ++ty)
+        for (uint32_t tx = 0; tx < tiles_x; ++tx) {
+            bool valid = false;
+            const uint32_t w = p.weigh(tx, ty, nullptr, &valid);
+            if (!valid) return;
+            if (w >= threshold) found.emplace_back(w, ty * tiles_x + tx);
+        }
+    std::sort(found.begin(), found.end(), [](const std::pair<uint32_t, uint32_t> &a, const std::pair<uint32_t, uint32_t> &b) {
+        return a.first != b.first ? a.first > b.first : a.second < b.second;
+    });
+    if (found.size() > cap) found.resize(cap);
+    if (found.size() < kProbeLongMinTiles) return;
+    s.long_bits.assign((n_tiles + 31u) / 32u, 0u);
+    for (const auto &f : found) {
+        s.long_tiles.push_back(f.second);
+        s.long_weights.push_back(f.first);
+        s.long_bits[f.second >> 5] |= 1u << (f.second & 31u);
+    }
 }
 
 
diff --git a/ray-tracer-rust_amd/csrc/scene_prep.h b/ray-tracer-rust_amd/csrc/scene_prep.h
--- a/ray-tracer-rust_amd/csrc/scene_prep.h
+++ b/ray-tracer-rust_amd/csrc/scene_prep.h
@@ -159,7 +159,18 @@
     uint32_t leaf_max = 4;
     uint32_t n_global = 0;
     std::vector<TriRec>   global_planes;
-};
+    std::vector<uint32_t> long_tiles, long_weights, long_bits;
+    float sample_lo[2] = {0.0f, 0.0f}, sample_hi[2] = {0.0f, 0.0f};
+};
+#ifndef RTX_PROBE_LONG_WEIGHT
+#define RTX_PROBE_LONG_WEIGHT 300
+#endif
+constexpr uint32_t kProbeLongWeight = RTX_PROBE_LONG_WEIGHT;
+constexpr uint32_t kProbeSplitMaxNodes = 1u << 16;
+constexpr uint32_t kProbeLongMinTiles = 8u;
+inline uint32_t probe_long_cap(uint32_t n_tiles) { return n_tiles / 32u < 1024u ? n_tiles / 32u : 1024u; }
+uint32_t probe_tile_weight(const PreparedScene &s, uint32_t tile_x, uint32_t tile_y, uint8_t *met, bool *valid);
+void predict_long_tiles(PreparedScene &s, uint32_t threshold);
 constexpr uint32_t kMaxGlobalPrims = 8u;
 constexpr uint64_t kMaxPrimitives = 1ull << 26;
 
diff --git a/ray-tracer-rust_amd/rtx.py b/ray-tracer-rust_amd/rtx.py
--- a/ray-tracer-rust_amd/rtx.py
+++ b/ray-tracer-rust_amd/rtx.py
@@ -186,6 +186,10 @@
     "rtx_debug_wave_profile": (C.c_int, [C.c_void_p, C.c_int, C.c_uint32, C.c_uint32, u64p, C.c_size_t, u32p, u32p]),
     "rtx_launch_timings": (C.c_int, [C.c_void_p, C.c_int, C.c_int, f32p, f32p]),
     "rtx_debug_tile_descs": (C.c_int, [C.c_void_p, C.c_int, u32p, C.c_size_t]),
+    "rtx_debug_probe_records": (C.c_int, [C.c_void_p, C.c_int, u32p, u32p, C.c_size_t]),
+    "rtx_scene_probe_long": (C.c_int, [C.c_void_p, u32p, u32p, C.c_size_t, u32p]),
+    "rtx_scene_probe_tile": (C.c_int, [C.c_void_p, C.c_uint32, C.c_uint32, u8p, u32p]),
+    "rtx_debug_probe_split": (C.c_int, [C.c_void_p, C.c_uint32]),
     "rtx_strerror": (C.c_char_p, [C.c_int]),
     "rtx_last_hip_error": (C.c_int, []),
     "rtx_scene_light_points": (C.c_int, [C.c_void_p, f32p]),
@@ -494,6 +498,41 @@
             raise RtxError(m, "rtx_debug_tile_descs")
         return out[:m]
 
+    def probe_records(self, device=0):
+        n = _lib.rtx_debug_probe_records(self._h, device, None, None, 0)
+        if n < 0:
+            raise RtxError(n, "rtx_debug_probe_records")
+        hits, slots = np.zeros((n, 768), np.uint32), np.zeros((n, 64), np.uint32)
+        m = _lib.rtx_debug_probe_records(self._h, device, hits.ctypes.data_as(u32p), slots.ctypes.data_as(u32p), n)
+        if m < 0:
+            raise RtxError(m, "rtx_debug_probe_records")
+        return hits[:m], slots[:m]
+
+    def probe_long(self):
+        n = _lib.rtx_scene_probe_long(self._h, None, None, 0, None)
+        if n < 0:
+            raise RtxError(n, "rtx_scene_probe_long")
+        tiles, weights, thr = np.zeros(n, np.uint32), np.zeros(n, np.uint32), C.c_uint32(0)
+        m = _lib.rtx_scene_probe_long(self._h, tiles.ctypes.data_as(u32p), weights.ctypes.data_as(u32p), n,
+                                      C.cast(C.byref(thr), u32p))
+        if m < 0:
+            raise RtxError(m, "rtx_scene_probe_long")
+        return tiles[:m], weights[:m], thr.value
+
+    def probe_tile(self, tile_x, tile_y):
+        met = np.zeros(self.info()["n_nodes"], np.uint8)
+        w = C.c_uint32(0)
+        rc = _lib.rtx_scene_probe_tile(self._h, tile_x, tile_y, met.ctypes.data_as(u8p), C.cast(C.byref(w), u32p))
+        if rc < 0:
+            raise RtxError(rc, "rtx_scene_probe_tile")
+        return w.value, met, bool(rc)
+
+    def debug_probe_split(self, mode):
+        n = _lib.rtx_debug_probe_split(self._h, mode)
+        if n < 0:
+            raise RtxError(n, "rtx_debug_probe_split")
+        return n
+
     def tiles_rows(self, first_tile, tile_stride, tile_rows):
         return _lib.rtx_tiles_rows(self._h, first_tile, tile_stride, tile_rows)
 
```

Result: faster. 141,000, median of 6 (+2.2%).
